# mgp25/OpenLTE

Measured on AMD Instinct MI355X. Metric: DL subframes/sec @20MHz 100RB 64QAM, full chain FFT->CE->demap->rate-unmatch->turbo(REF)->CRC (SURVEY 8d W4), higher is better.
Workload: dtype i8 IQ in, f32 FFT/CE/equaliser, i8 soft bits, i16 path metrics (differences exact modulo 2^16); 1 GPU; W4 full DL chain: 20 MHz/100 RB/64QAM, 9 allocations per subframe (8x12 PRB TBS 3240 + 1x4 PRB TBS 1064), 65536 subframes per GPU, int8 IQ in HBM; subframes_per_gpu=65536, N_ant=1, CFI=2, channel_estimate_form=compact, decoder=REF (reference-faithful, bit-exact), unique_subframes=96, streams_per_gpu=1

## Files before the change

### include/mi_lte.h

```cpp
#ifndef MI_LTE_H
#define MI_LTE_H

#include <stddef.h>
#include <stdint.h>

#ifdef __cplusplus
extern "C" {
#endif

#define MI_LTE_VERSION 100

typedef enum {
    MI_LTE_OK               = 0,
    MI_LTE_ERR_INVALID_ARG  = -1,
    MI_LTE_ERR_NO_DEVICE    = -2,
    MI_LTE_ERR_HIP          = -3,
    MI_LTE_ERR_UNSUPPORTED  = -4,
    MI_LTE_ERR_NOMEM        = -5
} mi_lte_status;

enum { MI_LTE_DECODE_SUCCESS = 0, MI_LTE_DECODE_INVALID_INPUTS = 1, MI_LTE_DECODE_FAIL = 2, MI_LTE_DECODE_INVALID_CRC = 3,
       MI_LTE_DECODE_INVALID_CONTENTS = 4 };

typedef struct mi_lte_ctx mi_lte_ctx;
// ... 53 lines not shown
    uint8_t  prb[2][112];
} mi_lte_pdsch_alloc;

typedef struct mi_lte_pdsch_plan mi_lte_pdsch_plan;
int      mi_lte_pdsch_plan_create(mi_lte_ctx *ctx, const mi_lte_dl_cfg *cfg, uint32_t N_pdcch_symbs,
                                  const mi_lte_pdsch_alloc *h_allocs, uint32_t n_alloc, mi_lte_pdsch_plan **out);
void     mi_lte_pdsch_plan_destroy(mi_lte_ctx *ctx, mi_lte_pdsch_plan *plan);
int      mi_lte_pdsch_plan_create_dynamic(mi_lte_ctx *ctx, const mi_lte_dl_cfg *cfg, uint32_t max_alloc, size_t max_soft_bytes,
                                          mi_lte_pdsch_plan **out);
int      mi_lte_pdsch_plan_assign(mi_lte_ctx *ctx, mi_lte_pdsch_plan *plan, uint32_t N_pdcch_symbs, const mi_lte_pdsch_alloc *h_allocs,
                                  uint32_t n_alloc);
uint32_t mi_lte_pdsch_plan_n_alloc(const mi_lte_pdsch_plan *plan);
int      mi_lte_pdsch_alloc_decodable(const mi_lte_dl_cfg *cfg, const mi_lte_pdsch_alloc *alloc, uint32_t N_pdcch_symbs);
int      mi_lte_pdsch_plan_set_decoder(mi_lte_pdsch_plan *plan, uint32_t mode , uint32_t n_iter, int qpp_spec);
int      mi_lte_pdsch_plan_set_output(mi_lte_pdsch_plan *plan, uint32_t packed);
uint32_t mi_lte_pdsch_plan_out_stride(const mi_lte_pdsch_plan *plan);
int      mi_lte_pdsch_decode_run(mi_lte_ctx *ctx, mi_lte_pdsch_plan *plan, const float *d_subframes,
                                 const uint32_t *d_subfr_num, const uint32_t *d_n_id_cell, uint8_t *d_out_bits,
                                 int32_t *d_status);
int      mi_lte_pdsch_plan_soft_bits(const mi_lte_pdsch_plan *plan, uint32_t alloc, const int8_t **d_e,
                                     const uint32_t **d_len);

typedef struct {
    uint32_t N_soft;
    uint32_t M_dl_harq;
} mi_lte_dlsch_cfg;

#define MI_LTE_DLSCH_MAX_CB 13
typedef struct {
    uint32_t C, K;
    uint32_t B;
    uint32_t N_cb, k0;
    uint32_t E[MI_LTE_DLSCH_MAX_CB];
    uint32_t off[MI_LTE_DLSCH_MAX_CB];
} mi_lte_dlsch_layout_t;

int mi_lte_dlsch_layout(uint32_t tbs, uint32_t G, uint32_t Q_m, uint32_t tx_mode, uint32_t rv, const mi_lte_dlsch_cfg *dlsch,
                        mi_lte_dlsch_layout_t *out);
int mi_lte_pdsch_plan_create_3gpp(mi_lte_ctx *ctx, const mi_lte_dl_cfg *cfg, uint32_t N_pdcch_symbs, const mi_lte_dlsch_cfg *dlsch,
                                  const mi_lte_pdsch_alloc *h_allocs, uint32_t n_alloc, mi_lte_pdsch_plan **out);
int mi_lte_pdsch_alloc_decodable_3gpp(const mi_lte_dl_cfg *cfg, const mi_lte_dlsch_cfg *dlsch, const mi_lte_pdsch_alloc *alloc,
                                      uint32_t N_pdcch_symbs);
int mi_lte_pdsch_plan_cb_soft(const mi_lte_pdsch_plan *plan, uint32_t alloc, const int8_t **d_blocks, uint32_t *C, uint32_t *K);
int mi_lte_pdsch_plan_cb_ok(const mi_lte_pdsch_plan *plan, const uint32_t **d_mask);

#define MI_LTE_DEMAP_REF    0u
#define MI_LTE_DEMAP_MAXLOG 1u
#define MI_LTE_DEMAP_AUTO_T 16
int mi_lte_pdsch_plan_set_demapper(mi_lte_pdsch_plan *plan, uint32_t mode, float gain);
int mi_lte_pdsch_plan_llr_gain(const mi_lte_pdsch_plan *plan, const float **d_gain);

typedef struct mi_lte_harq_pool mi_lte_harq_pool;
#define MI_LTE_HARQ_NONE     0xFFFFFFFFu
#define MI_LTE_HARQ_NEW_DATA 1u
typedef struct {
    uint32_t buf;
    uint32_t flags;
} mi_lte_harq_bind;
typedef struct {
    uint32_t tbs, C, K, N_cb;
    uint32_t n_tx;
    int32_t  status;
} mi_lte_harq_state;
size_t mi_lte_harq_buffer_bytes(uint32_t max_tbs);
int  mi_lte_harq_pool_create(mi_lte_ctx *ctx, uint32_t n_buf, uint32_t max_tbs, mi_lte_harq_pool **out);
void mi_lte_harq_pool_destroy(mi_lte_ctx *ctx, mi_lte_harq_pool *pool);
int  mi_lte_harq_pool_reset(mi_lte_ctx *ctx, mi_lte_harq_pool *pool, uint32_t buf);
int  mi_lte_pdsch_decode_run_harq(mi_lte_ctx *ctx, mi_lte_pdsch_plan *plan, mi_lte_harq_pool *pool, const mi_lte_harq_bind *h_bind,
                                  const float *d_subframes, const uint32_t *d_subfr_num, const uint32_t *d_n_id_cell, uint8_t *d_out_bits,
                                  int32_t *d_status);
int  mi_lte_harq_pool_soft(const mi_lte_harq_pool *pool, uint32_t buf, const int16_t **d_soft, const mi_lte_harq_state **d_state);

typedef enum { MI_LTE_TURBO_REF = 0, MI_LTE_TURBO_BCJR = 1, MI_LTE_TURBO_BCJR_BLOCK = 2, MI_LTE_TURBO_BCJR_EARLY = 3 } mi_lte_turbo_mode;
typedef enum { MI_LTE_SOFT_F32 = 0, MI_LTE_SOFT_I8 = 1, MI_LTE_SOFT_I16 = 2 } mi_lte_soft_type;

int mi_lte_turbo_decode_batch(mi_lte_ctx *ctx, const void *d_soft, mi_lte_soft_type soft_type, uint32_t K,
                              uint32_t n_cb, mi_lte_turbo_mode mode, uint32_t n_iter, int qpp_spec,
                              uint8_t *d_c_bits);

int mi_lte_turbo_early_exit_iterations(mi_lte_ctx *ctx, uint32_t *h_pair_iters, uint32_t max_pairs, uint32_t *n_pairs, uint32_t *n_iter);

int mi_lte_set_turbo_small_batch(mi_lte_ctx *ctx, uint32_t n_cb_max);
int mi_lte_set_turbo_merged(mi_lte_ctx *ctx, uint32_t on);

int mi_lte_rate_unmatch_turbo_batch(mi_lte_ctx *ctx, const float *d_e_bits, uint32_t N_e_bits, uint32_t D,
                                    uint32_t N_codeblocks, uint32_t tx_mode, uint32_t N_soft, uint32_t M_dl_harq,
                                    uint32_t chan_type, uint32_t rv_idx, uint32_t n_cb, float *d_d_bits);

size_t mi_lte_turbo_scratch_bytes(uint32_t K, uint32_t n_cb);
size_t mi_lte_turbo_bcjr_scratch_bytes(uint32_t K, uint32_t n_cb);

const char *mi_lte_last_kernels(const mi_lte_ctx *ctx);

size_t mi_lte_ul_subframe_floats(void);
int    mi_lte_ul_frontend_batch(mi_lte_ctx *ctx, const mi_lte_dl_cfg *cfg ,
                                const void *d_samples_a, const void *d_samples_b, const uint64_t *d_unit_start,
                                uint32_t n_units, float *d_subframes);

typedef struct {
    uint32_t group_assignment_pusch;
    uint32_t group_hopping_enabled;
    uint32_t sequence_hopping_enabled;
    uint32_t cyclic_shift;
    uint32_t cyclic_shift_dci;
} mi_lte_ul_cfg;

int mi_lte_ul_dmrs_pusch(const mi_lte_ul_cfg *ul, uint32_t N_id_cell, uint32_t N_subfr, uint32_t N_prb, float *h_dmrs_0_re,
                         float *h_dmrs_0_im, float *h_dmrs_1_re, float *h_dmrs_1_im);

typedef struct mi_lte_pusch_plan mi_lte_pusch_plan;
int      mi_lte_pusch_plan_create(mi_lte_ctx *ctx, const mi_lte_dl_cfg *cfg, const mi_lte_ul_cfg *ul,
                                  const uint32_t *h_unit_subfr_num, const uint32_t *h_unit_n_id_cell, uint32_t n_units,
                                  const mi_lte_pdsch_alloc *h_allocs, uint32_t n_alloc, mi_lte_pusch_plan **out);
void     mi_lte_pusch_plan_destroy(mi_lte_ctx *ctx, mi_lte_pusch_plan *plan);
uint32_t mi_lte_pusch_plan_out_stride(const mi_lte_pusch_plan *plan);
int      mi_lte_pusch_decode_run(mi_lte_ctx *ctx, mi_lte_pusch_plan *plan, const float *d_subframes, uint8_t *d_out_bits,
                                 int32_t *d_status);
int      mi_lte_pusch_plan_soft_bits(const mi_lte_pusch_plan *plan, uint32_t alloc, const int8_t **d_e, uint32_t *n_bits);

#define MI_LTE_ULSCH_N_SOFT 0xFFFFFFFFu
#define MI_LTE_ULSCH_M_HARQ 1u
int mi_lte_ulsch_layout(uint32_t tbs, uint32_t G, uint32_t Q_m, uint32_t rv, mi_lte_dlsch_layout_t *out);
int mi_lte_pusch_plan_create_3gpp(mi_lte_ctx *ctx, const mi_lte_dl_cfg *cfg, const mi_lte_ul_cfg *ul, const uint32_t *h_unit_subfr_num,
                                  const uint32_t *h_unit_n_id_cell, uint32_t n_units, const mi_lte_pdsch_alloc *h_allocs, uint32_t n_alloc,
                                  mi_lte_pusch_plan **out);
int mi_lte_pusch_plan_set_decoder(mi_lte_pusch_plan *plan, uint32_t mode, uint32_t n_iter, int qpp_spec);
int mi_lte_pusch_plan_set_output(mi_lte_pusch_plan *plan, uint32_t packed);
int mi_lte_pusch_plan_cb_soft(const mi_lte_pusch_plan *plan, uint32_t alloc, const int8_t **d_blocks, uint32_t *C, uint32_t *K);
int mi_lte_pusch_plan_cb_ok(const mi_lte_pusch_plan *plan, const uint32_t **d_mask);

typedef struct {
    uint8_t  O_ack, O_ri;
    uint16_t Qp_ack, Qp_ri;
    uint32_t Q_cqi;
} mi_lte_ulsch_uci;
enum { MI_LTE_UCI_ACK = 0, MI_LTE_UCI_RI = 1, MI_LTE_UCI_CQI = 2 };
int mi_lte_ulsch_uci_qprime(uint32_t kind, uint32_t O, uint32_t beta_x8, uint32_t M_sc_initial, uint32_t N_symb_initial, uint32_t sum_K_r,
                            uint32_t N_prb, uint32_t Qp_ri, uint32_t *Qp);
int mi_lte_ulsch_uci_G(uint32_t N_prb, uint32_t Q_m, const mi_lte_ulsch_uci *uci, uint32_t *G);
enum { MI_LTE_UCI_CELL_DATA = 0, MI_LTE_UCI_CELL_CQI = 1, MI_LTE_UCI_CELL_RI = 2, MI_LTE_UCI_CELL_ACK_DATA = 3, MI_LTE_UCI_CELL_ACK_CQI = 4 };
int mi_lte_ulsch_uci_map(uint32_t N_prb, uint32_t Q_m, const mi_lte_ulsch_uci *uci, uint8_t *kind , uint32_t *index );
typedef struct {
    uint8_t ack[2], ri[2];
    int32_t S_ack[3], S_ri[3];
} mi_lte_ulsch_uci_result;
int mi_lte_pusch_plan_create_3gpp_uci(mi_lte_ctx *ctx, const mi_lte_dl_cfg *cfg, const mi_lte_ul_cfg *ul, const uint32_t *h_unit_subfr_num,
                                      const uint32_t *h_unit_n_id_cell, uint32_t n_units, const mi_lte_pdsch_alloc *h_allocs, uint32_t n_alloc,
                                      const mi_lte_ulsch_uci *h_uci , mi_lte_pusch_plan **out);
int mi_lte_pusch_plan_uci_results(const mi_lte_pusch_plan *plan, const mi_lte_ulsch_uci_result **d_records);
int mi_lte_pusch_plan_cqi_soft(const mi_lte_pusch_plan *plan, uint32_t alloc, const int8_t **d_cqi, uint32_t *Q_cqi);
int mi_lte_pusch_plan_data_soft(const mi_lte_pusch_plan *plan, uint32_t alloc, const int8_t **d_data, uint32_t *G);

#define MI_LTE_CQI_MAX_BITS 128
enum { MI_LTE_CQI_NONE = 0, MI_LTE_CQI_NO_CRC = 1 , MI_LTE_CQI_CRC_OK = 2, MI_LTE_CQI_CRC_FAIL = 3 };
typedef struct {
    uint32_t O;
    uint32_t crc;
    int32_t  metric;
    int32_t  energy;
    uint32_t bits[4];
} mi_lte_cqi_result;
typedef struct { uint32_t off , Q_cqi, O, pad; } mi_lte_cqi_desc;
int mi_lte_cqi_encode(uint32_t O, const uint8_t *o_bits, uint32_t Q_cqi, uint8_t *q_bits );
int mi_lte_cqi_decode_batch(mi_lte_ctx *ctx, const int8_t *d_soft, const mi_lte_cqi_desc *d_desc, uint32_t n, mi_lte_cqi_result *d_out);
int mi_lte_pusch_plan_set_cqi_decode(mi_lte_pusch_plan *plan, const uint32_t *h_O_cqi );
int mi_lte_pusch_plan_cqi_results(const mi_lte_pusch_plan *plan, const mi_lte_cqi_result **d_records);
// ... 367 lines not shown
```

### openlte_amd/csrc/chain.hip

```cpp
#include <algorithm>
#include <cstring>
#include <type_traits>

#include "plan_core.hpp"
#include "phy_dev.hpp"
#include "demap_llr.h"

namespace {

constexpr int N_SC_MAX = 1200;

struct DemodGeom { uint32_t N_rb_dl, N_ant, cfi, sf_stride; };
__device__ __forceinline__ void sync_window(uint32_t N_rb_dl, uint32_t &first_sc, uint32_t &last_sc)
{
    switch (N_rb_dl) {
    case 6:  first_sc = 0;           last_sc = 71;          break;
    case 15: first_sc = 4 * 12 + 6;  last_sc = 11 * 12 - 7; break;
    case 25: first_sc = 9 * 12 + 6;  last_sc = 16 * 12 - 7; break;
    case 50: first_sc = 22 * 12;     last_sc = 28 * 12 - 1; break;
    case 75: first_sc = 34 * 12 + 6; last_sc = 41 * 12 - 7; break;
    default: first_sc = 47 * 12;     last_sc = 53 * 12 - 1; break;
    }
}
__device__ __forceinline__ uint32_t pdsch_mask(uint32_t N_ant, uint32_t cell, uint32_t sf, uint32_t L, uint32_t prb,
                                               uint32_t first_sc, uint32_t last_sc)
{
    const uint32_t l7 = L >= 7 ? L - 7 : L, c6 = cell % 6, c3 = cell % 3;
    uint32_t skip = 0;
    if (N_ant == 1) {
        if (l7 == 0) skip = 0x041u << c6;
        else if (l7 == 4) skip = 0x041u << ((c6 + 3) % 6);
    } else if (l7 == 0 || l7 == 4 || (N_ant == 4 && l7 == 1))
        skip = (0x249u << c3) & 0xFFFu;
    const bool win = (sf == 0 && L >= 7 && L <= 10) || ((sf == 0 || sf == 5) && (L == 5 || L == 6));
    const uint32_t s0 = prb * 12;
    if (win && last_sc >= s0 && first_sc <= s0 + 11) {
        const uint32_t lo = first_sc > s0 ? first_sc - s0 : 0u, hi = last_sc - s0 < 11u ? last_sc - s0 : 11u;
        skip |= ((2u << hi) - 1u) & ~((1u << lo) - 1u);
    }
    return ~skip & 0xFFFu;
}

__device__ __forceinline__ void pair_table_scan(uint2 *tab, const mi_lte_pdsch_alloc &al, uint32_t N_ant, uint32_t cell, uint32_t sf, uint32_t cfi,
                                                uint32_t n_pairs, uint32_t first_sc, uint32_t last_sc)
{
    const uint32_t N_prb = al.N_prb;
    const uint32_t ln = threadIdx.x, per = (n_pairs + 63) / 64, q0 = ln * per, q1 = min(q0 + per, n_pairs);
    const float r_prb = __builtin_amdgcn_rcpf((float)N_prb) * (1.0f + 0x1.8p-22f);
    uint32_t local = 0;
    for (uint32_t q = q0; q < q1; q++) {
        const uint32_t L = (uint32_t)((float)q * r_prb), prb = al.prb[L >= 7 ? 1 : 0][q - __umul24(L, N_prb)];
        const uint32_t m = L < cfi ? 0u : pdsch_mask(N_ant, cell, sf, L, prb, first_sc, last_sc);
        tab[q].y = m | ((L * N_SC_MAX + prb * 12) << 12);
        local += __popc(m);
    }
    uint32_t incl = local;
    for (int o = 1; o < 64; o <<= 1) {
        const uint32_t n = __shfl_up(incl, o);
        if ((int)ln >= o) incl += n;
    }
    uint32_t run = incl - local;
    for (uint32_t q = q0; q < q1; q++) {
        tab[q].x = run;
        run += __popc(tab[q].y & 0xFFFu);
    }
    if (ln == 63) tab[n_pairs] = make_uint2(incl, 0u);
}

template <bool ONE_PORT, bool COMPACT = false>
#ifndef DEMOD_WPE
#define DEMOD_WPE 8
#endif
#ifndef DEMOD_WPE_C
#define DEMOD_WPE_C 8
#endif
__global__ __launch_bounds__(256) __attribute__((amdgpu_waves_per_eu(COMPACT ? DEMOD_WPE_C : DEMOD_WPE, 8))) void k_pdsch_demod(const float *__restrict__ subframes, DemodGeom g,
                                                     const mi_lte_pdsch_alloc *__restrict__ allocs,
                                                     const uint32_t *__restrict__ subfr_num, const uint32_t *__restrict__ n_id_cell,
                                                     GoldTables gt, int8_t *__restrict__ e_base, const uint32_t *__restrict__ e_off,
                                                     uint32_t *__restrict__ e_len, uint32_t max_pairs, uint32_t max_words,
                                                     uint32_t e_lds_cap)
{
    extern __shared__ __attribute__((aligned(16))) uint32_t smu[];
    __shared__ uint2 qam_lut[64];
    const uint32_t a_idx = blockIdx.x;
    const mi_lte_pdsch_alloc &al = allocs[a_idx];
    const uint32_t unit = al.unit, sf = subfr_num[unit], cell = n_id_cell[unit], N_ant = ONE_PORT ? 1u : g.N_ant, N_prb = al.N_prb;
    const uint32_t Qm = al.mod_type == 3 ? 6 : al.mod_type == 2 ? 4 : al.mod_type == 1 ? 2 : 1;
    uint2    *tab = reinterpret_cast<uint2 *>(smu);
    uint32_t *cw  = smu + ((2 * (max_pairs + 1) + 3u) & ~3u);
    uint32_t first_sc, last_sc;
    sync_window(g.N_rb_dl, first_sc, last_sc);

    const uint32_t cfi = al.n_pdcch_symbs ? al.n_pdcch_symbs : g.cfi;
    const uint32_t n_pairs = 14 * N_prb, pair0 = cfi * N_prb;
    const uint32_t c_init = ((al.rnti << 14) | (0u << 13) | (sf << 9) | cell) & 0x7FFFFFFFu;
    if (threadIdx.x < 64) pair_table_scan(tab, al, N_ant, cell, sf, cfi, n_pairs, first_sc, last_sc);
    else {
        const uint32_t n_words_ub = ((n_pairs - pair0) * 12 * Qm + 31) / 32;
        if (threadIdx.x < 128) qam_lut[threadIdx.x - 64] = qam_lut_entry(threadIdx.x - 64);
        for (uint32_t w = threadIdx.x - 64; w <= n_words_ub; w += blockDim.x - 64) cw[w] = gold_word(gt, c_init, w);
    }
    __syncthreads();
    const uint32_t M_ap = tab[n_pairs].x;
    const uint32_t n_grp = M_ap >> (N_ant >> 1), M_symb = n_grp * N_ant, N_bits = M_symb * Qm;
    if (threadIdx.x == 0) e_len[a_idx] = N_bits;

    const float *base = subframes + (size_t)unit * g.sf_stride;
    const float *y_re_p = base, *y_im_p = base + 16 * N_SC_MAX;
    const float *h_re_p = base + 2 * 16 * N_SC_MAX, *h_im_p = h_re_p + (size_t)N_ant * 16 * N_SC_MAX;
    int8_t *e = e_base + (size_t)e_off[a_idx] * 64;
    auto locate = [&](uint32_t idx) -> uint32_t {
        uint32_t lo = pair0, hi = n_pairs;
        while (hi - lo > 1) {
            const uint32_t mid = (lo + hi) >> 1;
            if (tab[mid].x <= idx) lo = mid; else hi = mid;
        }
        const uint2 t = tab[lo];
        uint32_t r = idx - t.x, m = t.y & 0xFFFu;
        for (; r; r--) m &= m - 1;
        return (t.y >> 12) + (uint32_t)__builtin_ctz(m);
    };
    int8_t    *e_lds  = reinterpret_cast<int8_t *>(cw + max_words);
    const bool via_lds = N_bits <= e_lds_cap;
    auto run = [&](auto modc) {
    constexpr uint32_t MOD = decltype(modc)::value, QM = MOD == 3 ? 6 : MOD == 2 ? 4 : MOD == 1 ? 2 : 1;
    constexpr bool     QAM = MOD >= 2;
    auto put_bits = [&](auto *dst, uint32_t idx, const int8_t (&b)[6]) {
        const uint32_t n0 = idx * QM, w = n0 >> 5, sh = n0 & 31;
        const uint32_t c = __builtin_amdgcn_alignbit(cw[w + 1], cw[w], sh);
        if (QM == 1) dst[n0] = (c & 1u) ? (int8_t)-b[0] : b[0];
        else {
#pragma unroll
            for (uint32_t k = 0; k < 6; k += 2)
                if (k < QM) {
                    const int lo = ((c >> k) & 1u) ? -b[k] : b[k], hi = ((c >> (k + 1)) & 1u) ? -b[k + 1] : b[k + 1];
                    *reinterpret_cast<uint16_t *>(dst + n0 + k) = (uint16_t)((lo & 0xFF) | ((hi & 0xFF) << 8));
                }
        }
    };
    auto put_qam = [&](auto *dst, uint32_t idx, uint32_t neg) {
        const uint32_t n0 = QM == 4 ? idx << 2 : __umul24(idx, 6u), w = n0 >> 5, sh = n0 & 31;
        const uint32_t c  = __builtin_amdgcn_alignbit(cw[w + 1], cw[w], sh);
        const uint2    v  = qam_lut[(neg ^ c) & (QM == 4 ? 15u : 63u)];
        if (QM == 4) *reinterpret_cast<uint32_t *>(dst + n0) = v.x;
        else {
            *reinterpret_cast<uint16_t *>(dst + n0)     = (uint16_t)v.x;
            *reinterpret_cast<uint16_t *>(dst + n0 + 2) = (uint16_t)(v.x >> 16);
            *reinterpret_cast<uint16_t *>(dst + n0 + 4) = (uint16_t)v.y;
        }
    };
    auto put_symbol = [&](auto *dst, uint32_t idx, float nr, float ni, float den) {
        if constexpr (QAM) put_qam(dst, idx, qam_neg_bits_nodiv<MOD>(nr, ni, den));
        else {
            int8_t b[6] = {0, 0, 0, 0, 0, 0};
            demap_symbol<true>(nr / den, ni / den, MOD, b);
            put_bits(dst, idx, b);
        }
    };
    if (ONE_PORT && COMPACT) {
        constexpr uint32_t ROW = N_SC_MAX * 4, Y_IM = 16 * ROW, H_M = 32 * ROW, H_A = 48 * ROW;
        const uint32_t per_slot = N_prb * 12, n_items = 2 * per_slot;
        const auto rsrc = __builtin_amdgcn_make_buffer_rsrc(const_cast<float *>(base), 0, (int)(g.sf_stride * 4u), 0x00020000);
        auto ld = [&](uint32_t row, uint32_t off) { return __builtin_bit_cast(float, __builtin_amdgcn_raw_buffer_load_b32(rsrc, (int)off, (int)row, 0)); };
        auto body = [&](auto *dst) {
            for (uint32_t item = threadIdx.x; item < n_items; item += blockDim.x) {
                const uint32_t s = item >= per_slot ? 1u : 0u, r = item - s * per_slot, i = __umul24(r, 43691u) >> 19, j = r - ((i << 3) + (i << 2));
                const uint32_t bit = 1u << j, below = bit - 1u;
                const uint2   *tp = tab + (s ? 7 * N_prb : 0u) + i;
                const uint2    t0 = *tp;
                const uint32_t vy = ((t0.y >> 12) + j) << 2;
                const uint32_t vk = vy - s * (7 * ROW), vh = vk + s * (2 * ROW);
                const float M0 = ld(H_M, vh), M1 = ld(H_M + ROW, vh), M2 = ld(H_M + 2 * ROW, vh);
                const float P0 = ld(H_A, vh), P1 = ld(H_A + ROW, vh), P2 = ld(H_A + 2 * ROW, vh);
                const float Q0 = ld(H_A, vk), Q1 = ld(H_A + ROW, vk);
                float yr[7], yi[7];
#pragma unroll
                for (int t = 0; t < 7; t++) { yr[t] = ld(t * ROW, vy); yi[t] = ld(Y_IM + t * ROW, vy); }
                float m[7], a[7];
                m[0] = M0; a[0] = P0; m[4] = M1; a[4] = P1;
                float W0 = P0;
                if (s) W0 = wrap_phase_rare(P0, wrap_phase_rare(Q1, Q0));
                {
                    const float fm = (M1 - M0) / 4, W1 = wrap_phase_rare(P1, W0);
                    const float fa = wrap_phase_rare(W1 - W0, 0.0f) / 4;
                    float cm = M1, ca = W1;
#pragma unroll
                    for (int z = 3; z > 0; z--) { cm -= fm; ca -= fa; m[z] = cm; a[z] = ca; }
                    const float gm = div3(M2 - M1), W2 = wrap_phase_rare(P2, W1);
                    const float ga = div3(wrap_phase_rare(W2 - W1, 0.0f));
                    cm = M2; ca = W2;
#pragma unroll
                    for (int z = 6; z > 4; z--) { cm -= gm; ca -= ga; m[z] = cm; a[z] = ca; }
                }
#pragma unroll
                for (int t = 0; t < 7; t++) {
                    const uint2 pr = t ? tp[t * N_prb] : t0;
                    if (!(pr.y & bit)) continue;
                    const uint32_t idx = pr.x + __popc(pr.y & below);
                    float sn, cs;
                    ce_sincos(a[t], sn, cs);
                    const float mm = m[t], hr = mm * cs, hi = mm * sn;
                    const float hn = hr * hr + hi * hi;
                    put_symbol(dst, idx, yr[t] * hr + yi[t] * hi, yi[t] * hr - yr[t] * hi, hn);
                }
            }
        };
        if (via_lds) body(e_lds); else body(e);
    } else if (ONE_PORT) {
        constexpr int UNR = 4;
        const uint32_t q_thr = threadIdx.x / 12, j = threadIdx.x - 12 * q_thr, below = (1u << j) - 1u;
        const bool     lane_on = threadIdx.x < 252;
        auto body = [&](auto *dst) {
            for (uint32_t qb = pair0; qb < n_pairs; qb += 21 * UNR) {
                float    yr[UNR], yi[UNR], hr[UNR], hi[UNR];
                uint32_t idx[UNR];
                bool     on[UNR];
#pragma unroll
                for (int r = 0; r < UNR; r++) {
                    const uint32_t q = qb + 21 * r + q_thr;
                    const bool     in = lane_on && q < n_pairs;
                    const uint2    pr = tab[in ? q : 0u];
                    on[r]  = in && ((pr.y >> j) & 1u);
                    idx[r] = pr.x + __popc(pr.y & below);
                    const uint32_t ob = on[r] ? ((pr.y >> 12) + j) << 2 : 0u;
                    yr[r] = *reinterpret_cast<const float *>(reinterpret_cast<const char *>(y_re_p) + ob);
                    yi[r] = *reinterpret_cast<const float *>(reinterpret_cast<const char *>(y_im_p) + ob);
                    hr[r] = *reinterpret_cast<const float *>(reinterpret_cast<const char *>(h_re_p) + ob);
                    hi[r] = *reinterpret_cast<const float *>(reinterpret_cast<const char *>(h_im_p) + ob);
                }
#pragma unroll
                for (int r = 0; r < UNR; r++) {
                    if (!on[r]) continue;
                    const float hn = hr[r] * hr[r] + hi[r] * hi[r];
                    put_symbol(dst, idx[r], yr[r] * hr[r] + yi[r] * hi[r], yi[r] * hr[r] - yr[r] * hi[r], hn);
                }
            }
        };
        if (via_lds) body(e_lds); else body(e);
    } else
    for (uint32_t i = threadIdx.x; i < n_grp; i += blockDim.x) {
        float n_re[4], n_im[4], den[4];
        if (N_ant == 2) {
            const uint32_t p0 = locate(2 * i), p1 = locate(2 * i + 1);
            const float y0r = y_re_p[p0], y0i = y_im_p[p0], y1r = y_re_p[p1], y1i = y_im_p[p1];
            const float h0r = h_re_p[p0], h0i = h_im_p[p0], h1r = h_re_p[16 * N_SC_MAX + p0], h1i = h_im_p[16 * N_SC_MAX + p0];
            const float a0 = h0r * h0r + h0i * h0i, a1 = h1r * h1r + h1i * h1i;
            const float hn = sqrtf(a0 * a0 + a1 * a1);
            den[0] = den[1] = hn;
            n_re[0] = h0r * y0r + h0i * y0i + h1r * y1r + h1i * y1i;
            n_im[0] = h0r * y0i - h0i * y0r - h1r * y1i + h1i * y1r;
            n_re[1] = -h1r * y0r - h1i * y0i + h0r * y1r + h0i * y1i;
            n_im[1] = h1r * y0i - h1i * y0r + h0r * y1i - h0i * y1r;
        } else {
            const uint32_t p0 = locate(4 * i), p1 = locate(4 * i + 1), p2 = locate(4 * i + 2), p3 = locate(4 * i + 3);
            const size_t   ps = 16 * N_SC_MAX;
            const float y0r = y_re_p[p0], y0i = y_im_p[p0], y1r = y_re_p[p1], y1i = y_im_p[p1];
            const float y2r = y_re_p[p2], y2i = y_im_p[p2], y3r = y_re_p[p3], y3i = y_im_p[p3];
            const float h0r = h_re_p[p0], h0i = h_im_p[p0], h2r = h_re_p[2 * ps + p0], h2i = h_im_p[2 * ps + p0];
            const float h1r = h_re_p[ps + p2], h1i = h_im_p[ps + p2], h3r = h_re_p[3 * ps + p2], h3i = h_im_p[3 * ps + p2];
            const float a0 = h0r * h0r + h0i * h0i, a1 = h1r * h1r + h1i * h1i, a2 = h2r * h2r + h2i * h2i, a3 = h3r * h3r + h3i * h3i;
            const float n02 = sqrtf(a0 * a0 + a2 * a2), n13 = sqrtf(a1 * a1 + a3 * a3);
            den[0] = den[1] = n02; den[2] = den[3] = n13;
            n_re[0] = h0r * y0r + h0i * y0i + h2r * y1r + h2i * y1i;
            n_im[0] = h0r * y0i - h0i * y0r - h2r * y1i + h2i * y1r;
            n_re[1] = -h2r * y0r - h2i * y0i + h0r * y1r + h0i * y1i;
            n_im[1] = -(-h2r * y0i + h2i * y0r - h0r * y1i + h0i * y1r);
            n_re[2] = h1r * y2r + h1i * y2i + h3r * y3r + h3i * y3i;
            n_im[2] = h1r * y2i - h1i * y2r - h3r * y3i + h3i * y3r;
            n_re[3] = -h3r * y2r - h3i * y2i + h1r * y3r + h1i * y3i;
            n_im[3] = -(-h3r * y2i + h3i * y2r - h1r * y3i + h1i * y3r);
        }
        for (uint32_t p = 0; p < N_ant; p++) {
            if (via_lds) put_symbol(e_lds, i * N_ant + p, n_re[p], n_im[p], den[p]);
            else         put_symbol(e, i * N_ant + p, n_re[p], n_im[p], den[p]);
        }
    }
    };
    switch (al.mod_type) {
    case 0:  run(std::integral_constant<uint32_t, 0>{}); break;
    case 1:  run(std::integral_constant<uint32_t, 1>{}); break;
    case 2:  run(std::integral_constant<uint32_t, 2>{}); break;
    default: run(std::integral_constant<uint32_t, 3>{}); break;
    }
    if (via_lds) {
        __syncthreads();
        const uint32_t nq = (N_bits + 15) >> 4;
        for (uint32_t w = threadIdx.x; w < nq; w += blockDim.x) reinterpret_cast<uint4 *>(e)[w] = reinterpret_cast<const uint4 *>(e_lds)[w];
    }
}


__global__ __launch_bounds__(256) void k_pdsch_demod_llr(const float *__restrict__ subframes, DemodGeom g, const mi_lte_pdsch_alloc *__restrict__ allocs,
                                                         const uint32_t *__restrict__ subfr_num, const uint32_t *__restrict__ n_id_cell, GoldTables gt,
                                                         int8_t *__restrict__ e_base, const uint32_t *__restrict__ e_off, uint32_t *__restrict__ e_len,
                                                         uint32_t max_pairs, uint32_t max_words, uint32_t e_lds_cap, float gain, float auto_t,
                                                         float *__restrict__ llr_gain)
{
    extern __shared__ __attribute__((aligned(16))) uint32_t smu[];
    __shared__ double w_wave[4];
    const uint32_t a_idx = blockIdx.x;
    const mi_lte_pdsch_alloc &al = allocs[a_idx];
    const uint32_t unit = al.unit, sf = subfr_num[unit], cell = n_id_cell[unit], N_prb = al.N_prb;
    const uint32_t Qm = al.mod_type == 3 ? 6 : al.mod_type == 2 ? 4 : 2;
    uint2    *tab = reinterpret_cast<uint2 *>(smu);
    uint32_t *cw  = smu + ((2 * (max_pairs + 1) + 3u) & ~3u);
    uint32_t first_sc, last_sc;
    sync_window(g.N_rb_dl, first_sc, last_sc);
    const uint32_t cfi = al.n_pdcch_symbs ? al.n_pdcch_symbs : g.cfi;
    const uint32_t n_pairs = 14 * N_prb, pair0 = cfi * N_prb;
    const uint32_t c_init = ((al.rnti << 14) | (0u << 13) | (sf << 9) | cell) & 0x7FFFFFFFu;
    if (threadIdx.x < 64) pair_table_scan(tab, al, 1u, cell, sf, cfi, n_pairs, first_sc, last_sc);
    else {
        const uint32_t n_words_ub = ((n_pairs - pair0) * 12 * Qm + 31) / 32;
        for (uint32_t w = threadIdx.x - 64; w <= n_words_ub; w += blockDim.x - 64) cw[w] = gold_word(gt, c_init, w);
    }
    __syncthreads();
    const uint32_t M_symb = tab[n_pairs].x, N_bits = M_symb * Qm;
    if (threadIdx.x == 0) e_len[a_idx] = N_bits;

    const float *base = subframes + (size_t)unit * g.sf_stride;
    const char  *y_re_p = reinterpret_cast<const char *>(base), *y_im_p = y_re_p + 16 * N_SC_MAX * 4;
    const char  *h_re_p = y_im_p + 16 * N_SC_MAX * 4, *h_im_p = h_re_p + 16 * N_SC_MAX * 4;
    constexpr int  UNR = 4;
    const uint32_t q_thr = threadIdx.x / 12, j = threadIdx.x - 12 * q_thr, below = (1u << j) - 1u;
    const bool     lane_on = threadIdx.x < 252;
    auto element = [&](uint32_t q, uint32_t &ob, uint32_t &idx) __attribute__((always_inline)) -> bool {
        const bool  in = lane_on && q < n_pairs;
        const uint2 pr = tab[in ? q : 0u];
        const bool  on = in && ((pr.y >> j) & 1u);
        idx = pr.x + __popc(pr.y & below);
        ob  = on ? ((pr.y >> 12) + j) << 2 : 0u;
        return on;
    };
    double gd = (double)gain;
    if (gain == 0.0f) {
        double part = 0.0;
        for (uint32_t qb = pair0; qb < n_pairs; qb += 21 * UNR) {
            float hr[UNR], hi[UNR];
            bool  on[UNR];
#pragma unroll
            for (int r = 0; r < UNR; r++) {
                uint32_t ob, idx;
                on[r] = element(qb + 21 * r + q_thr, ob, idx);
                hr[r] = *reinterpret_cast<const float *>(h_re_p + ob);
                hi[r] = *reinterpret_cast<const float *>(h_im_p + ob);
            }
#pragma unroll
            for (int r = 0; r < UNR; r++)
                if (on[r]) part += (double)hr[r] * hr[r] + (double)hi[r] * hi[r];
        }
        for (int o = 32; o; o >>= 1) part += __shfl_xor(part, o);
        if ((threadIdx.x & 63u) == 0) w_wave[threadIdx.x >> 6] = part;
        __syncthreads();
        const double wbar = (((w_wave[0] + w_wave[1]) + w_wave[2]) + w_wave[3]) / (double)M_symb;
        const double a4 = al.mod_type == 3 ? 4.0 / 42 : al.mod_type == 2 ? 4.0 / 10 : 2.0;
        const float  gf = (float)((double)auto_t / (a4 * wbar));
        gd = (wbar > 0.0 && fabsf(gf) <= 3.4028234e38f) ? (double)gf : 0.0;
    }
    if (threadIdx.x == 0) llr_gain[a_idx] = (float)gd;

    int8_t    *e      = e_base + (size_t)e_off[a_idx] * 64;
    int8_t    *e_lds  = reinterpret_cast<int8_t *>(cw + max_words);
    const bool via_lds = N_bits <= e_lds_cap;
    auto run = [&](auto modc, auto *dst) __attribute__((always_inline)) {
        constexpr uint32_t MOD = decltype(modc)::value, QM = MOD == 3 ? 6 : MOD == 2 ? 4 : 2;
        for (uint32_t qb = pair0; qb < n_pairs; qb += 21 * UNR) {
            float    yr[UNR], yi[UNR], hr[UNR], hi[UNR];
            uint32_t idx[UNR];
            bool     on[UNR];
#pragma unroll
            for (int r = 0; r < UNR; r++) {
                uint32_t ob;
                on[r] = element(qb + 21 * r + q_thr, ob, idx[r]);
                yr[r] = *reinterpret_cast<const float *>(y_re_p + ob);
                yi[r] = *reinterpret_cast<const float *>(y_im_p + ob);
                hr[r] = *reinterpret_cast<const float *>(h_re_p + ob);
                hi[r] = *reinterpret_cast<const float *>(h_im_p + ob);
            }
#pragma unroll
            for (int r = 0; r < UNR; r++) {
                if (!on[r]) continue;
                const double Yr = yr[r], Yi = yi[r], Hr = hr[r], Hi = hi[r];
                const double w = Hr * Hr + Hi * Hi;
                double li[3], lq[3];
                llr_axis<MOD>(Yr * Hr + Yi * Hi, w, li);
                llr_axis<MOD>(Yi * Hr - Yr * Hi, w, lq);
                const uint32_t n0 = idx[r] * QM, c = __builtin_amdgcn_alignbit(cw[(n0 >> 5) + 1], cw[n0 >> 5], n0 & 31);
#pragma unroll
                for (uint32_t k = 0; k < QM; k += 2) {
                    const int vi = llr_byte(gd, li[k >> 1]), vq = llr_byte(gd, lq[k >> 1]);
                    const int lo = ((c >> k) & 1u) ? -vi : vi, hi8 = ((c >> (k + 1)) & 1u) ? -vq : vq;
                    *reinterpret_cast<uint16_t *>(dst + n0 + k) = (uint16_t)((lo & 0xFF) | ((hi8 & 0xFF) << 8));
                }
            }
        }
    };
    auto per_mod = [&](auto *dst) __attribute__((always_inline)) {
        switch (al.mod_type) {
        case 1:  run(std::integral_constant<uint32_t, 1>{}, dst); break;
        case 2:  run(std::integral_constant<uint32_t, 2>{}, dst); break;
        default: run(std::integral_constant<uint32_t, 3>{}, dst); break;
        }
    };
    if (via_lds) {
        per_mod(e_lds);
        __syncthreads();
        const uint32_t nq = (N_bits + 15) >> 4;
        for (uint32_t w = threadIdx.x; w < nq; w += blockDim.x) reinterpret_cast<uint4 *>(e)[w] = reinterpret_cast<const uint4 *>(e_lds)[w];
    } else
        per_mod(e);
}

}


struct mi_lte_pdsch_plan {
    mi_lte_dl_cfg cfg;
    MiPlanCore    core;
    uint32_t      decoder = MI_LTE_TURBO_REF, n_iter = 8;
    int           qpp_spec = 0;
    int8_t       *d_bcjr_soft = nullptr;
    uint8_t      *d_bcjr_bits = nullptr;
    size_t        bcjr_soft_cap = 0, bcjr_bits_cap = 0;
    uint32_t      cfi = 0, max_pairs = 0, max_words = 0, max_tbs = 0;
    bool          dynamic = false, wide = false;
    bool          mapped = false;
    void       *h_stage = nullptr;
    hipEvent_t  staged = nullptr;
    std::vector<uint8_t>  h_row;
    std::vector<uint32_t> h_e_bits;
    MiDlsch3   *g3 = nullptr;
    uint32_t    demap = MI_LTE_DEMAP_REF;
    float       demap_gain = 0.0f, *d_llr_gain = nullptr;
};

static void plan_set_stride(mi_lte_pdsch_plan *pl)
{
    pl->core.out_stride = mi_out_stride((pl->dynamic || pl->wide) ? 6120u : pl->max_tbs, pl->core.packed != 0);
}

static int plan_layout(mi_lte_ctx *ctx, mi_lte_pdsch_plan *pl, uint32_t N_pdcch_symbs, const mi_lte_pdsch_alloc *h_allocs, uint32_t n_alloc,
                       std::vector<uint32_t> *cb_alloc, bool prbs_checked = false)
{
    std::vector<uint8_t>  &row    = pl->h_row;
    std::vector<uint32_t> &e_bits = pl->h_e_bits;
    row.resize(n_alloc);
    e_bits.resize(n_alloc);
    const mi_lte_dl_cfg *cfg = &pl->cfg;
    pl->cfi          = N_pdcch_symbs;
    pl->core.n_alloc = n_alloc;
    pl->max_pairs = pl->max_words = pl->max_tbs = 0;
    pl->core.groups.clear();
    for (uint32_t a = 0; a < n_alloc; a++) {
        const mi_lte_pdsch_alloc &al = h_allocs[a];
        const int      r   = cb_alloc ? mi_qpp_row_at_least(al.tbs + 24) : 0;
        const uint32_t cfi = al.n_pdcch_symbs ? al.n_pdcch_symbs : N_pdcch_symbs;
        if (r < 0 || al.N_prb == 0 || al.N_prb > cfg->N_rb_dl || al.mod_type > 3 || cfi < 1 || cfi > 4) {
            ctx->err = "allocation outside the single-code-block envelope (tbs + 24 > 6144) or malformed";
            return MI_LTE_ERR_UNSUPPORTED;
        }
        for (uint32_t s = 0; s < 2 && !prbs_checked; s++)
            for (uint32_t i = 0; i < al.N_prb; i++)
                if (al.prb[s][i] >= cfg->N_rb_dl) {
                    ctx->err = "allocation names a resource block outside the carrier";
                    return MI_LTE_ERR_INVALID_ARG;
                }
        row[a]      = (uint8_t)r;
        pl->max_tbs = std::max(pl->max_tbs, al.tbs);
        const uint32_t Qm = al.mod_type == 3 ? 6 : al.mod_type == 2 ? 4 : al.mod_type == 1 ? 2 : 1;
        const uint32_t pairs = (14 - cfi) * al.N_prb, e_max = pairs * 12 * Qm;
        pl->max_pairs = std::max(pl->max_pairs, 14 * al.N_prb);
        pl->max_words = std::max(pl->max_words, (e_max + 31) / 32);
        e_bits[a]     = e_max;
    }
    if (pl->max_words > 4095) {
        ctx->err = "allocation larger than the scrambling table";
        return MI_LTE_ERR_UNSUPPORTED;
    }
    pl->core.e_bytes = mi_plan_soft_layout(e_bits.data(), n_alloc, pl->core.h_e_off);
    plan_set_stride(pl);
    if (cb_alloc) mi_plan_group(row.data(), nullptr, e_bits.data(), n_alloc, pl->core.groups, *cb_alloc);
    return MI_LTE_OK;
}

extern "C" {

void mi_lte_pdsch_plan_destroy(mi_lte_ctx *ctx, mi_lte_pdsch_plan *pl);

int mi_lte_pdsch_plan_create(mi_lte_ctx *ctx, const mi_lte_dl_cfg *cfg, uint32_t N_pdcch_symbs,
                             const mi_lte_pdsch_alloc *h_allocs, uint32_t n_alloc, mi_lte_pdsch_plan **out)
{
    if (!ctx || !cfg || !h_allocs || !out || n_alloc == 0 || N_pdcch_symbs < 1 || N_pdcch_symbs > 4) return MI_LTE_ERR_INVALID_ARG;
    if (!(cfg->N_ant == 1 || cfg->N_ant == 2 || cfg->N_ant == 4)) return MI_LTE_ERR_INVALID_ARG;
    if ((cfg->sample_format & MI_LTE_CE_COMPACT) && cfg->N_ant != 1) { ctx->err = "MI_LTE_CE_COMPACT: single-port cells only"; return MI_LTE_ERR_UNSUPPORTED; }
    MI_HIP_CHECK(ctx, hipSetDevice(ctx->device));
    auto *pl      = new mi_lte_pdsch_plan();
    auto  guard   = on_fail([&] { (void)hipStreamSynchronize(ctx->stream); mi_lte_pdsch_plan_destroy(nullptr, pl); });
    pl->cfg       = *cfg;
    std::vector<uint32_t> cb_alloc;
    int rc = plan_layout(ctx, pl, N_pdcch_symbs, h_allocs, n_alloc, &cb_alloc);
    if (rc != MI_LTE_OK) return rc;
    MI_HIP_CHECK(ctx, pl->core.allocate(n_alloc, pl->core.e_bytes));
    MI_H2D(ctx, pl->core.d_allocs, h_allocs, sizeof(mi_lte_pdsch_alloc) * n_alloc);
    MI_H2D(ctx, pl->core.d_e_off, pl->core.h_e_off.data(), sizeof(uint32_t) * n_alloc);
    MI_H2D(ctx, pl->core.d_cb_alloc, cb_alloc.data(), sizeof(uint32_t) * n_alloc);
    MI_HIP_CHECK(ctx, mi_stream_wait_polling(ctx));
    guard.armed = false;
    *out = pl;
    return MI_LTE_OK;
}

int mi_lte_pdsch_plan_create_dynamic(mi_lte_ctx *ctx, const mi_lte_dl_cfg *cfg, uint32_t max_alloc, size_t max_soft_bytes, mi_lte_pdsch_plan **out)
{
    if (!ctx || !cfg || !out || max_alloc == 0) return MI_LTE_ERR_INVALID_ARG;
    if (!(cfg->N_ant == 1 || cfg->N_ant == 2 || cfg->N_ant == 4)) return MI_LTE_ERR_INVALID_ARG;
    if ((cfg->sample_format & MI_LTE_CE_COMPACT) && cfg->N_ant != 1) { ctx->err = "MI_LTE_CE_COMPACT: single-port cells only"; return MI_LTE_ERR_UNSUPPORTED; }
    MI_HIP_CHECK(ctx, hipSetDevice(ctx->device));
    auto *pl    = new mi_lte_pdsch_plan();
    auto  guard = on_fail([&] { mi_lte_pdsch_plan_destroy(nullptr, pl); });
    pl->cfg     = *cfg;
    pl->dynamic = true;
    max_alloc = (max_alloc + 3u) & ~3u;
    MI_HIP_CHECK(ctx, pl->core.allocate(max_alloc, (max_soft_bytes + 63) & ~(size_t)63));
    MI_HIP_CHECK(ctx, hipHostMalloc(&pl->h_stage, (sizeof(mi_lte_pdsch_alloc) + 2 * sizeof(uint32_t)) * (size_t)max_alloc, hipHostMallocDefault));
    MI_HIP_CHECK(ctx, hipEventCreateWithFlags(&pl->staged, hipEventDisableTiming));
    guard.armed = false;
    *out = pl;
    return MI_LTE_OK;
}
}

int mi_pdsch_plan_create_mapped(mi_lte_ctx *ctx, const mi_lte_dl_cfg *cfg, uint32_t max_alloc, size_t max_soft_bytes, mi_lte_pdsch_plan **out)
{
    if (!ctx || !cfg || !out || max_alloc == 0 || max_alloc > 64) return MI_LTE_ERR_INVALID_ARG;
    if (!(cfg->N_ant == 1 || cfg->N_ant == 2 || cfg->N_ant == 4) || (cfg->sample_format & MI_LTE_CE_COMPACT)) return MI_LTE_ERR_INVALID_ARG;
    MI_HIP_CHECK(ctx, hipSetDevice(ctx->device));
    auto *pl    = new mi_lte_pdsch_plan();
    auto  guard = on_fail([&] { mi_lte_pdsch_plan_destroy(nullptr, pl); });
    pl->cfg     = *cfg;
    pl->dynamic = pl->mapped = true;
    MI_HIP_CHECK(ctx, hipHostMalloc(&pl->h_stage, (sizeof(mi_lte_pdsch_alloc) + 2 * sizeof(uint32_t)) * (size_t)max_alloc, hipHostMallocMapped | hipHostMallocCoherent));
    void *d_stage = nullptr;
    MI_HIP_CHECK(ctx, hipHostGetDevicePointer(&d_stage, pl->h_stage, 0));
    MI_HIP_CHECK(ctx, pl->core.allocate(max_alloc, (max_soft_bytes + 63) & ~(size_t)63, d_stage));
    guard.armed = false;
    *out = pl;
    return MI_LTE_OK;
}

static bool alloc_geometry_ok(const mi_lte_dl_cfg *cfg, const mi_lte_pdsch_alloc *al, uint32_t N_pdcch_symbs)
{
    const uint32_t cfi = al->n_pdcch_symbs ? al->n_pdcch_symbs : N_pdcch_symbs;
    if (al->N_prb == 0 || al->N_prb > cfg->N_rb_dl || al->N_prb > 110 || al->mod_type > 3 || cfi < 1 || cfi > 4) return false;
    if ((14 - cfi) * al->N_prb * 12 * (al->mod_type == 3 ? 6u : al->mod_type == 2 ? 4u : al->mod_type == 1 ? 2u : 1u) > 4095u * 32u) return false;
    for (uint32_t s = 0; s < 2; s++)
// ... 76 lines not shown
    memcpy(so, pl->core.h_e_off.data(), sizeof(uint32_t) * n_alloc);
    memcpy(sc, cb_alloc.data(), sizeof(uint32_t) * n_alloc);
    if (pl->mapped) return MI_LTE_OK;
    MI_HIP_CHECK(ctx, hipMemcpyAsync(pl->core.d_allocs, sa, sizeof(mi_lte_pdsch_alloc) * n_alloc, hipMemcpyHostToDevice, ctx->stream));
    MI_HIP_CHECK(ctx, hipMemcpyAsync(pl->core.d_e_off, so, sizeof(uint32_t) * n_alloc, hipMemcpyHostToDevice, ctx->stream));
    MI_HIP_CHECK(ctx, hipMemcpyAsync(pl->core.d_cb_alloc, sc, sizeof(uint32_t) * n_alloc, hipMemcpyHostToDevice, ctx->stream));
    MI_HIP_CHECK(ctx, hipEventRecord(pl->staged, ctx->stream));
    return MI_LTE_OK;
}

uint32_t mi_lte_pdsch_plan_n_alloc(const mi_lte_pdsch_plan *pl) { return pl ? pl->core.n_alloc : 0; }
}

int mi_pdsch_plan_assign_slice(mi_lte_ctx *ctx, mi_lte_pdsch_plan *pl, uint32_t N_pdcch_symbs, const mi_lte_pdsch_alloc *h_src, uint32_t n_alloc, uint32_t unit0,
                               std::vector<uint32_t> *refused, hipStream_t copy_stream)
{
    if (!ctx || !pl || !pl->dynamic || pl->mapped || !h_src || n_alloc == 0 || N_pdcch_symbs < 1 || N_pdcch_symbs > 4) return MI_LTE_ERR_INVALID_ARG;
    const hipStream_t cs = copy_stream ? copy_stream : ctx->stream;
    if (n_alloc > pl->core.cap_alloc) { ctx->err = "more allocations than the dynamic plan was created for"; return MI_LTE_ERR_INVALID_ARG; }
    MI_HIP_CHECK(ctx, hipSetDevice(ctx->device));
    MI_HIP_CHECK(ctx, hipEventSynchronize(pl->staged));
    auto *sa = (mi_lte_pdsch_alloc *)pl->h_stage;
    auto *so = (uint32_t *)(sa + pl->core.cap_alloc), *sc = so + pl->core.cap_alloc;
    for (uint32_t i = 0; i < n_alloc; i++) {
        mi_lte_pdsch_alloc &a = sa[i];
        a = h_src[i];
        a.unit -= unit0;
        if (!mi_lte_pdsch_alloc_decodable(&pl->cfg, &a, N_pdcch_symbs)) {
            a.N_prb = 1; a.prb[0][0] = a.prb[1][0] = 0; a.mod_type = 1; a.tbs = 16; a.rv_idx = 0; a.tx_mode = pl->cfg.N_ant == 1 ? 1 : 2;
            if (a.n_pdcch_symbs > 4) a.n_pdcch_symbs = 0;
            if (refused) refused->push_back(i);
        }
    }
    std::vector<uint32_t> cb_alloc;
    int rc = plan_layout(ctx, pl, N_pdcch_symbs, sa, n_alloc, &cb_alloc, true);
    if (rc != MI_LTE_OK) { pl->core.n_alloc = 0; return rc; }
    if (pl->core.e_bytes > pl->core.cap_e_bytes) { pl->core.n_alloc = 0; ctx->err = "more soft bits than the dynamic plan was created for"; return MI_LTE_ERR_INVALID_ARG; }
    memcpy(so, pl->core.h_e_off.data(), sizeof(uint32_t) * n_alloc);
    memcpy(sc, cb_alloc.data(), sizeof(uint32_t) * n_alloc);
    static const bool slice_by_engine = getenv("MI_LTE_SLICE_COPY_COMMANDS") != nullptr;
    if (slice_by_engine) {
        MI_HIP_CHECK(ctx, hipMemcpyAsync(pl->core.d_allocs, sa, sizeof(mi_lte_pdsch_alloc) * n_alloc, hipMemcpyHostToDevice, cs));
        MI_HIP_CHECK(ctx, hipMemcpyAsync(pl->core.d_e_off, so, sizeof(uint32_t) * n_alloc, hipMemcpyHostToDevice, cs));
        MI_HIP_CHECK(ctx, hipMemcpyAsync(pl->core.d_cb_alloc, sc, sizeof(uint32_t) * n_alloc, hipMemcpyHostToDevice, cs));
    } else {
        const MiCopySeg segs[3] = {{pl->core.d_allocs, sa, sizeof(mi_lte_pdsch_alloc) * n_alloc}, {pl->core.d_e_off, so, sizeof(uint32_t) * n_alloc}, {pl->core.d_cb_alloc, sc, sizeof(uint32_t) * n_alloc}};
        MI_HIP_CHECK(ctx, mi_pinned_segments_to_device(ctx, segs, 3, cs));
    }
    MI_HIP_CHECK(ctx, hipEventRecord(pl->staged, cs));
    return MI_LTE_OK;
}
void mi_pdsch_plan_wide_stride(mi_lte_pdsch_plan *pl) { pl->wide = true; plan_set_stride(pl); }
extern "C" {

void mi_lte_pdsch_plan_destroy(mi_lte_ctx *ctx, mi_lte_pdsch_plan *pl)
{
    if (!pl) return;
    if (ctx) {
        (void)hipSetDevice(ctx->device);
        (void)hipStreamSynchronize(ctx->stream);
    }
    pl->core.release();
    if (pl->d_bcjr_soft) (void)hipFree(pl->d_bcjr_soft);
    if (pl->d_bcjr_bits) (void)hipFree(pl->d_bcjr_bits);
    if (pl->d_llr_gain) (void)hipFree(pl->d_llr_gain);
    if (pl->h_stage) (void)hipHostFree(pl->h_stage);
    if (pl->staged) (void)hipEventDestroy(pl->staged);
    mi_dlsch3_free(pl->g3);
    delete pl;
}

uint32_t mi_lte_pdsch_plan_out_stride(const mi_lte_pdsch_plan *pl) { return pl ? pl->core.out_stride : 0; }

int mi_lte_model_atan2f(const float *h_y, const float *h_x, float *h_out, size_t n)
{
    if (!h_y || !h_x || !h_out) return MI_LTE_ERR_INVALID_ARG;
    for (size_t i = 0; i < n; i++) h_out[i] = ref_atan2f(h_y[i], h_x[i]);
    return MI_LTE_OK;
}

int mi_lte_pdsch_plan_soft_bits(const mi_lte_pdsch_plan *pl, uint32_t alloc, const int8_t **d_e, const uint32_t **d_len)
{
    if (!pl || alloc >= pl->core.n_alloc || !d_e || !d_len) return MI_LTE_ERR_INVALID_ARG;
    *d_e   = pl->core.d_e + (size_t)pl->core.h_e_off[alloc] * 64;
    *d_len = pl->core.d_e_len + alloc;
    return MI_LTE_OK;
}

int mi_lte_pdsch_plan_set_decoder(mi_lte_pdsch_plan *pl, uint32_t mode, uint32_t n_iter, int qpp_spec)
{
    const bool bcjr = mi_is_bcjr(mode);
    if (!pl || !(mode == MI_LTE_TURBO_REF || bcjr) || (bcjr && (n_iter == 0 || n_iter > 64))) return MI_LTE_ERR_INVALID_ARG;
    if (pl->g3 && mode == MI_LTE_TURBO_REF) return MI_LTE_ERR_UNSUPPORTED;
    if (pl->g3 && !qpp_spec) return MI_LTE_ERR_INVALID_ARG;
    pl->decoder = mode; pl->n_iter = n_iter; pl->qpp_spec = qpp_spec;
    return MI_LTE_OK;
}

int mi_lte_pdsch_plan_set_demapper(mi_lte_pdsch_plan *pl, uint32_t mode, float gain)
{
    if (!pl || mode > MI_LTE_DEMAP_MAXLOG) return MI_LTE_ERR_INVALID_ARG;
    if (mode == MI_LTE_DEMAP_REF) { pl->demap = MI_LTE_DEMAP_REF; return MI_LTE_OK; }
    if (!(gain >= 0.0f) || gain > 3.4028234e38f) return MI_LTE_ERR_INVALID_ARG;
    if (!pl->g3 || (pl->cfg.sample_format & MI_LTE_CE_COMPACT)) return MI_LTE_ERR_UNSUPPORTED;
    pl->demap = mode; pl->demap_gain = gain;
    return MI_LTE_OK;
}

int mi_lte_pdsch_plan_llr_gain(const mi_lte_pdsch_plan *pl, const float **d_gain)
{
    if (!pl || !d_gain || !pl->d_llr_gain) return MI_LTE_ERR_INVALID_ARG;
    *d_gain = pl->d_llr_gain;
    return MI_LTE_OK;
}

int mi_lte_pdsch_plan_set_output(mi_lte_pdsch_plan *pl, uint32_t packed)
{
    if (!pl) return MI_LTE_ERR_INVALID_ARG;
    pl->core.packed = packed ? 1u : 0u;
    plan_set_stride(pl);
    return MI_LTE_OK;
}

}

static int pdsch_demod(mi_lte_ctx *ctx, mi_lte_pdsch_plan *pl, const float *d_subframes, const uint32_t *d_subfr_num, const uint32_t *d_n_id_cell)
{
    MI_HIP_CHECK(ctx, hipSetDevice(ctx->device));
    int rc = mi_ctx_gold_tables(ctx);
    if (rc != MI_LTE_OK) return rc;
    DemodGeom  g{pl->cfg.N_rb_dl, pl->cfg.N_ant, pl->cfi, (uint32_t)mi_lte_subframe_floats(pl->cfg.N_ant)};
    GoldTables gt{ctx->d_gold_x1, ctx->d_gold_x2b, ctx->gold_words};
    const uint32_t words_al = (pl->max_words + 1u + 3u) & ~3u, e_bytes = (pl->max_words * 32 + 63u) & ~63u;
    const uint32_t e_cap = (e_bytes <= 32 * 1024) ? e_bytes : 0;
    const uint32_t pairs_al = ((2 * (pl->max_pairs + 1) + 3u) & ~3u);
    const size_t lds = sizeof(uint32_t) * ((size_t)pairs_al + words_al) + e_cap;
    uint32_t threads = 256;
    if (const char *ev = getenv("MI_LTE_PDSCH_THREADS")) {
        const int t = atoi(ev);
        if (t >= 64 && t <= 256 && t % 64 == 0) threads = (uint32_t)t;
    }
    auto launch = [&](auto kernel) {
        MI_LAUNCH(ctx, "k_pdsch_demod", kernel, dim3(pl->core.n_alloc), dim3(threads), lds, d_subframes, g, pl->core.d_allocs, d_subfr_num, d_n_id_cell, gt,
                  pl->core.d_e, pl->core.d_e_off, pl->core.d_e_len, pl->max_pairs, words_al, e_cap);
    };
    if (pl->demap == MI_LTE_DEMAP_MAXLOG) {
        float auto_t = (float)MI_LTE_DEMAP_AUTO_T;
        if (const char *ev = getenv("MI_LTE_DEMAP_AUTO_T")) {
            const float t = (float)atof(ev);
            if (t >= 1.0f && t <= 127.0f) auto_t = t;
        }
        MI_LAUNCH(ctx, "k_pdsch_demod_llr", k_pdsch_demod_llr, dim3(pl->core.n_alloc), dim3(256), lds, d_subframes, g, pl->core.d_allocs, d_subfr_num,
                  d_n_id_cell, gt, pl->core.d_e, pl->core.d_e_off, pl->core.d_e_len, pl->max_pairs, words_al, e_cap, pl->demap_gain, auto_t, pl->d_llr_gain);
    } else if (g.N_ant == 1 && (pl->cfg.sample_format & MI_LTE_CE_COMPACT)) launch(k_pdsch_demod<true, true>);
    else if (g.N_ant == 1) launch(k_pdsch_demod<true>);
    else launch(k_pdsch_demod<false>);
    MI_HIP_CHECK(ctx, hipGetLastError());
    return MI_LTE_OK;
}

static int pdsch_run(mi_lte_ctx *ctx, mi_lte_pdsch_plan *pl, mi_lte_harq_pool *pool, const mi_lte_harq_bind *h_bind, const float *d_subframes,
                     const uint32_t *d_subfr_num, const uint32_t *d_n_id_cell, uint8_t *d_out_bits, int32_t *d_status)
{
    if (!ctx || !pl || !d_subframes || !d_subfr_num || !d_n_id_cell || !d_out_bits || !d_status) return MI_LTE_ERR_INVALID_ARG;
    int rc;
    if (pool) {
        if (!pl->g3) { ctx->err = "HARQ soft combining needs a plan in the 3GPP transport-block mode"; return MI_LTE_ERR_UNSUPPORTED; }
        if ((rc = mi_dlsch3_harq_check(ctx, pl->g3, pool, h_bind)) != MI_LTE_OK) return rc;
    }
    if (pl->core.n_alloc == 0) { ctx->err = "the dynamic plan holds no allocations (mi_lte_pdsch_plan_assign)"; return MI_LTE_ERR_INVALID_ARG; }
    if ((rc = pdsch_demod(ctx, pl, d_subframes, d_subfr_num, d_n_id_cell)) != MI_LTE_OK) return rc;
    const MiDecodeIO io = pl->core.io(d_out_bits, d_status, false);
    if (pl->g3) {
        rc = mi_dlsch3_run(ctx, pl->g3, pool, h_bind, io, pl->decoder, pl->n_iter);
        if (rc == MI_LTE_OK && pl->demap == MI_LTE_DEMAP_MAXLOG) ctx->last_kernels.replace(0, strlen("k_pdsch_demod"), "k_pdsch_demod_llr");
        return rc;
    }
    if (!mi_is_bcjr(pl->decoder)) {
        rc = mi_turbo_ref_dispatch(ctx, pl->core.groups.data(), (uint32_t)pl->core.groups.size(), io, &pl->core.multi);
        if (rc != MI_LTE_OK) return rc;
        ctx->last_kernels.insert(0, "k_pdsch_demod:1,");
        return MI_LTE_OK;
    }
    size_t soft = 0, bits = 0;
    for (auto &gr : pl->core.groups) { soft = std::max(soft, (size_t)gr.n_cb * 3 * (gr.K + 4)); bits = std::max(bits, (size_t)gr.n_cb * gr.K); }
    if (soft > pl->bcjr_soft_cap || bits > pl->bcjr_bits_cap) {
        MI_HIP_CHECK(ctx, hipStreamSynchronize(ctx->stream));
        if (pl->d_bcjr_soft) (void)hipFree(pl->d_bcjr_soft);
        if (pl->d_bcjr_bits) (void)hipFree(pl->d_bcjr_bits);
        pl->d_bcjr_soft = nullptr; pl->d_bcjr_bits = nullptr;
        MI_HIP_CHECK(ctx, hipMalloc((void **)&pl->d_bcjr_soft, soft));
        MI_HIP_CHECK(ctx, hipMalloc((void **)&pl->d_bcjr_bits, bits));
        pl->bcjr_soft_cap = soft; pl->bcjr_bits_cap = bits;
    }
    for (auto &gr : pl->core.groups) {
        rc = mi_turbo_bcjr_group(ctx, gr, io, pl->d_bcjr_soft, pl->d_bcjr_bits, pl->decoder, pl->n_iter, pl->qpp_spec);
        if (rc != MI_LTE_OK) return rc;
    }
    ctx->last_kernels = pl->decoder == MI_LTE_TURBO_BCJR_BLOCK ? "k_pdsch_demod:1,k_rm_to_i8,k_bcjr_block,k_crc_finish per block size"
                                                               : "k_pdsch_demod:1,k_cb_desc,k_rm_bcjr_prep,k_bcjr_half,k_bcjr_final,k_crc_finish per block size";
    return MI_LTE_OK;
}

extern "C" {

int mi_lte_pdsch_decode_run(mi_lte_ctx *ctx, mi_lte_pdsch_plan *pl, const float *d_subframes, const uint32_t *d_subfr_num,
                            const uint32_t *d_n_id_cell, uint8_t *d_out_bits, int32_t *d_status)
{
    return pdsch_run(ctx, pl, nullptr, nullptr, d_subframes, d_subfr_num, d_n_id_cell, d_out_bits, d_status);
}

int mi_lte_pdsch_decode_run_harq(mi_lte_ctx *ctx, mi_lte_pdsch_plan *pl, mi_lte_harq_pool *pool, const mi_lte_harq_bind *h_bind, const float *d_subframes,
                                 const uint32_t *d_subfr_num, const uint32_t *d_n_id_cell, uint8_t *d_out_bits, int32_t *d_status)
{
    if (!pool || !h_bind) return MI_LTE_ERR_INVALID_ARG;
    return pdsch_run(ctx, pl, pool, h_bind, d_subframes, d_subfr_num, d_n_id_cell, d_out_bits, d_status);
}

}
```

### openlte_amd/csrc/ctx.cc

```cpp
#include <cmath>

#include <chrono>
#include <cstdlib>

#include <algorithm>

#include "ctx.hpp"
#include "build_id.h"

#include <cstring>

#include "lte_tables.h"

extern "C" {

int mi_lte_version(void) { return MI_LTE_VERSION; }
const char *mi_lte_build_id(void) { return MI_LTE_BUILD_ID; }

int mi_lte_device_count(void)
{
    int n = 0;
    if (hipGetDeviceCount(&n) != hipSuccess) return 0;
    return n;
}

int mi_lte_ctx_create(int device, mi_lte_ctx **out)
{
    if (!out) return MI_LTE_ERR_INVALID_ARG;
    *out  = nullptr;
    int n = mi_lte_device_count();
    if (n <= 0 || device < 0 || device >= n) {
        fprintf(stderr, "mi_lte: no usable HIP device %d (found %d); this library has no CPU fallback\n", device, n);
        return MI_LTE_ERR_NO_DEVICE;
    }
    mi_lte_ctx *ctx = new mi_lte_ctx();
    ctx->device     = device;
    if (const char *e = getenv("MI_LTE_NO_MERGED_DECODE")) ctx->merged_decode = atoi(e) == 0;
    hipDeviceProp_t prop;
    if (hipSetDevice(device) != hipSuccess || hipGetDeviceProperties(&prop, device) != hipSuccess) {
        delete ctx;
        return MI_LTE_ERR_HIP;
    }
    ctx->dev_name = std::string(prop.name) + " (" + prop.gcnArchName + ")";
    if (std::strncmp(prop.gcnArchName, "gfx950", 6) != 0) {
        fprintf(stderr, "mi_lte: device %d is %s, but the kernels are built for gfx950 only\n", device, prop.gcnArchName);
        delete ctx;
        return MI_LTE_ERR_NO_DEVICE;
    }
    if (hipStreamCreateWithFlags(&ctx->stream, hipStreamNonBlocking) != hipSuccess || hipEventCreate(&ctx->ev0) != hipSuccess ||
        hipEventCreate(&ctx->ev1) != hipSuccess) {
        delete ctx;
        return MI_LTE_ERR_HIP;
    }
    *out = ctx;
    return MI_LTE_OK;
}

void mi_lte_ctx_destroy(mi_lte_ctx *ctx)
{
    if (!ctx) return;
    (void)hipSetDevice(ctx->device);
    (void)hipStreamSynchronize(ctx->stream);
    if (ctx->host_cache_free) ctx->host_cache_free(ctx);
    for (void *p : ctx->owned) (void)hipFree(p);
    for (hipEvent_t e : ctx->prof_pool) (void)hipEventDestroy(e);
    if (ctx->scratch) (void)hipFree(ctx->scratch);
    if (ctx->h_small) (void)hipHostFree(ctx->h_small);
    if (ctx->h_bounce) (void)hipHostFree(ctx->h_bounce);
    for (int k = 0; k < 2; k++)
        if (ctx->ev_bounce[k]) (void)hipEventDestroy(ctx->ev_bounce[k]);
    if (ctx->h_flag) (void)hipHostFree(ctx->h_flag);
    if (ctx->ev0) (void)hipEventDestroy(ctx->ev0);
    if (ctx->ev1) (void)hipEventDestroy(ctx->ev1);
    if (ctx->stream) (void)hipStreamDestroy(ctx->stream);
    delete ctx;
}

int mi_lte_set_turbo_small_batch(mi_lte_ctx *ctx, uint32_t n_cb_max)
{
    if (!ctx) return MI_LTE_ERR_INVALID_ARG;
    ctx->siso_small_max = n_cb_max;
    return MI_LTE_OK;
}

int mi_lte_set_turbo_merged(mi_lte_ctx *ctx, uint32_t on)
{
    if (!ctx) return MI_LTE_ERR_INVALID_ARG;
    ctx->merged_decode = on != 0;
    return MI_LTE_OK;
}

const char *mi_lte_last_error(const mi_lte_ctx *ctx) { return ctx ? ctx->err.c_str() : "null context"; }
const char *mi_lte_device_name(const mi_lte_ctx *ctx) { return ctx ? ctx->dev_name.c_str() : ""; }
void       *mi_lte_stream(const mi_lte_ctx *ctx) { return ctx ? (void *)ctx->stream : nullptr; }
const char *mi_lte_last_kernels(const mi_lte_ctx *ctx) { return ctx ? ctx->last_kernels.c_str() : ""; }

int mi_lte_malloc(mi_lte_ctx *ctx, size_t bytes, void **d_ptr)
{
    if (!ctx || !d_ptr) return MI_LTE_ERR_INVALID_ARG;
    MI_HIP_CHECK(ctx, hipSetDevice(ctx->device));
    MI_HIP_CHECK(ctx, hipMalloc(d_ptr, bytes ? bytes : 1));
    return MI_LTE_OK;
}
int mi_lte_free(mi_lte_ctx *ctx, void *d_ptr)
{
    if (!ctx) return MI_LTE_ERR_INVALID_ARG;
    MI_HIP_CHECK(ctx, hipSetDevice(ctx->device));
    MI_HIP_CHECK(ctx, hipStreamSynchronize(ctx->stream));
    MI_HIP_CHECK(ctx, hipFree(d_ptr));
    return MI_LTE_OK;
}
int mi_lte_memset(mi_lte_ctx *ctx, void *d_ptr, int value, size_t bytes)
{
    if (!ctx) return MI_LTE_ERR_INVALID_ARG;
    MI_HIP_CHECK(ctx, hipMemsetAsync(d_ptr, value, bytes, ctx->stream));
    return MI_LTE_OK;
}
}
namespace {
typedef uint32_t mi_u32x4 __attribute__((ext_vector_type(4)));
template <bool NT> __global__ void k_copy16(const mi_u32x4 *__restrict__ src, mi_u32x4 *__restrict__ dst, size_t n)
{
    const size_t i = (size_t)blockIdx.x * blockDim.x + threadIdx.x;
    if (i >= n) return;
    if (NT) __builtin_nontemporal_store(__builtin_nontemporal_load(src + i), dst + i);
    else dst[i] = src[i];
}
__global__ void k_copy16_loop(const mi_u32x4 *__restrict__ src, mi_u32x4 *__restrict__ dst, size_t n)
{
    for (size_t i = (size_t)blockIdx.x * blockDim.x + threadIdx.x; i < n; i += (size_t)gridDim.x * blockDim.x) dst[i] = src[i];
}
}
extern "C" {
int mi_lte_device_copy_rate(mi_lte_ctx *ctx, size_t bytes, uint32_t reps, double *gb_per_s)
{
    if (!ctx || !gb_per_s || bytes < 16 || (bytes & 15) || reps == 0) return MI_LTE_ERR_INVALID_ARG;
    MI_HIP_CHECK(ctx, hipSetDevice(ctx->device));
    mi_u32x4 *a = nullptr, *b = nullptr;
    auto      guard = on_fail([&] { (void)hipStreamSynchronize(ctx->stream); (void)hipFree(a); (void)hipFree(b); });
    MI_HIP_CHECK(ctx, hipMalloc((void **)&a, bytes));
    MI_HIP_CHECK(ctx, hipMalloc((void **)&b, bytes));
    MI_HIP_CHECK(ctx, hipMemsetAsync(a, 0x5A, bytes, ctx->stream));
    const size_t n = bytes / 16;
    if ((n + 255) / 256 > 0x7FFFFFFFull) return MI_LTE_ERR_INVALID_ARG;
    const dim3 block(256), grid_all((unsigned)((n + 255) / 256)), grid_loop((unsigned)std::min<size_t>((n + 255) / 256, 256 * 32));
    double     best = 0.0;
    for (int shape = 0; shape < 3; shape++) {
        auto launch = [&](const mi_u32x4 *s, mi_u32x4 *d) {
            if (shape == 0) hipLaunchKernelGGL(k_copy16<false>, grid_all, block, 0, ctx->stream, s, d, n);
            else if (shape == 1) hipLaunchKernelGGL(k_copy16<true>, grid_all, block, 0, ctx->stream, s, d, n);
            else hipLaunchKernelGGL(k_copy16_loop, grid_loop, block, 0, ctx->stream, s, d, n);
        };
        launch(a, b);
        MI_HIP_CHECK(ctx, hipEventRecord(ctx->ev0, ctx->stream));
        for (uint32_t r = 0; r < reps; r++) launch((r & 1) ? b : a, (r & 1) ? a : b);
        MI_HIP_CHECK(ctx, hipEventRecord(ctx->ev1, ctx->stream));
        MI_HIP_CHECK(ctx, hipEventSynchronize(ctx->ev1));
        MI_HIP_CHECK(ctx, hipGetLastError());
        float ms = 0.f;
        MI_HIP_CHECK(ctx, hipEventElapsedTime(&ms, ctx->ev0, ctx->ev1));
        const double r = 2.0 * (double)bytes * reps / ((double)ms * 1e-3) / 1e9;
        ctx->copy_rates[shape] = r;
        best = std::max(best, r);
    }
    *gb_per_s = best;
    guard.armed = false;
    (void)hipFree(a); (void)hipFree(b);
    return MI_LTE_OK;
}
int mi_lte_device_copy_rates(const mi_lte_ctx *ctx, double *out3)
{
// ... 417 lines not shown
```

### openlte_amd/csrc/ctx.hpp

```cpp
#pragma once

#include <hip/hip_runtime.h>

#include <cstdint>
#include <cstdio>
#include <map>
#include <string>
#include <vector>

#include "../../include/mi_lte.h"
#include "turbo_plan.hpp"

struct TurboTables {
    uint16_t *d_pi  = nullptr;
    uint16_t *d_inv = nullptr;
    uint16_t *d_inv2 = nullptr;
    uint32_t *d_pi_row = nullptr, *d_inv_row = nullptr;
};

struct RmTables {
    uint16_t *d_tabs = nullptr;
    uint32_t *d_nnn  = nullptr;
};

enum : uint32_t { MI_FFT_TWC_P2 = 0, MI_FFT_TWC_P3 = 32, MI_FFT_TWC_L2048 = 288, MI_FFT_TWC_L1024 = 1312, MI_FFT_TWC_L256 = 1824, MI_FFT_TWC_L128 = 1952,
                  MI_FFT_TWC_X2 = 2016, MI_FFT_TWC_X3 = 2048,
                  MI_FFT_TWC_TOTAL = 2560 };

constexpr uint32_t MI_CRC_TAB_BIAS = 8;

struct mi_lte_ctx {
    int                device = -1;
    hipStream_t        stream = nullptr;
    hipEvent_t         ev0 = nullptr, ev1 = nullptr;
    std::string        err;
    std::string        dev_name;
    std::string        last_kernels;
    double             copy_rates[3] = {0, 0, 0};
    void              *scratch       = nullptr;
    size_t             scratch_bytes = 0;
    uint32_t          *h_flag = nullptr, *d_flag = nullptr;
    uint32_t           flag_seq = 0;
    uint32_t *bcjr_early_buf = nullptr; size_t bcjr_early_cap = 0;
    struct { uint32_t *chg; uint32_t n_pairs, n_iter, n_cb; } bcjr_early = {nullptr, 0, 0, 0};
    bool               bcjr_block_lds_set = false;
    uint32_t           siso_small_max = 4096;
    bool               merged_decode = true;
    void              *h_small = nullptr, *d_small = nullptr;
    void              *h_bounce = nullptr, *d_bounce = nullptr;
    hipEvent_t         ev_bounce[2] = {nullptr, nullptr};
    bool               bounce_failed = false;
    std::map<uint64_t, TurboTables> turbo_tables;
    std::map<uint32_t, RmTables>    rm_tables;
    std::vector<void *> owned;

    uint32_t *d_gold_x1 = nullptr, *d_gold_x2b = nullptr;
    uint32_t  gold_words = 0;
    void     *d_pusch_shapes = nullptr;

    float2   *d_fft_tw  = nullptr;
    uint32_t *d_crc_tab = nullptr;
    float2   *d_prach_tab = nullptr;
    float2   *d_prach_tab4 = nullptr;

    bool                                   prof_on = false, prof_armed = false;
    std::vector<hipEvent_t>                prof_pool;
    size_t                                 prof_used = 0;
    std::vector<std::pair<const char *, size_t>> prof_recs;
    std::string                            prof_report;

    void *host_cache = nullptr;
    void (*host_cache_free)(mi_lte_ctx *) = nullptr;
};

void mi_prof_begin(mi_lte_ctx *ctx, const char *name);
void mi_prof_end(mi_lte_ctx *ctx);

#define MI_LAUNCH(ctx, name, kernel, grid, block, shmem, ...)                                         \
    do {                                                                                             \
        mi_prof_begin((ctx), (name));                                                                \
        hipLaunchKernelGGL(kernel, grid, block, shmem, (ctx)->stream, __VA_ARGS__);                  \
        mi_prof_end((ctx));                                                                          \
    } while (0)

#define MI_HIP_CHECK(ctx, call)                                                                      \
    do {                                                                                             \
        hipError_t e_ = (call);                                                                      \
        if (e_ != hipSuccess) {                                                                      \
            (ctx)->err = std::string(#call) + ": " + hipGetErrorString(e_);                          \
            return MI_LTE_ERR_HIP;                                                                   \
        }                                                                                            \
    } while (0)

#define MI_H2D(ctx, d, h, n) do { const int rc_ = mi_lte_memcpy_h2d((ctx), (d), (h), (n)); if (rc_ != MI_LTE_OK) return rc_; } while (0)
#define MI_D2H(ctx, h, d, n) do { const int rc_ = mi_lte_memcpy_d2h((ctx), (h), (d), (n)); if (rc_ != MI_LTE_OK) return rc_; } while (0)

template <typename F> struct OnFail {
    F    f;
    bool armed = true;
    ~OnFail() { if (armed) f(); }
};
template <typename F> OnFail<F> on_fail(F f) { return OnFail<F>{f}; }

int   mi_ctx_reserve_scratch(mi_lte_ctx *ctx, size_t bytes);
hipError_t mi_pinned_to_device(mi_lte_ctx *ctx, void *d_dst, const void *h_pinned, size_t bytes, hipStream_t stream = nullptr);
hipError_t mi_device_to_pinned(mi_lte_ctx *ctx, void *h_pinned, const void *d_src, size_t bytes);
struct MiCopySeg { void *dst; const void *src; size_t bytes; };
hipError_t mi_pinned_segments_to_device(mi_lte_ctx *ctx, const MiCopySeg *segs, uint32_t n_seg, hipStream_t stream);
constexpr size_t MI_SMALL_BYTES = 64 * 1024;
int   mi_ctx_small_results(mi_lte_ctx *ctx, size_t bytes, void **h, void **d);
hipError_t mi_stream_wait(mi_lte_ctx *ctx, size_t n_units);
hipError_t mi_stream_wait_polling(mi_lte_ctx *ctx);
int   mi_ctx_gold_tables(mi_lte_ctx *ctx);
int   mi_ctx_crc_table(mi_lte_ctx *ctx);
int   mi_ctx_fft_twiddles(mi_lte_ctx *ctx);
struct MiMultiCache { void *d_tab = nullptr; size_t cap = 0; std::vector<MiKGroup> built_for; MiMultiGeom geom; };
void  mi_multi_cache_free(MiMultiCache *cache);
int   mi_ctx_turbo_tables(mi_lte_ctx *ctx, uint32_t K, int spec, TurboTables *out);
struct mi_lte_pdsch_plan;
int   mi_pdsch_plan_create_mapped(mi_lte_ctx *ctx, const mi_lte_dl_cfg *cfg, uint32_t max_alloc, size_t max_soft_bytes, mi_lte_pdsch_plan **out);
int   mi_pdsch_plan_assign_slice(mi_lte_ctx *ctx, mi_lte_pdsch_plan *pl, uint32_t N_pdcch_symbs, const mi_lte_pdsch_alloc *h_src, uint32_t n_alloc, uint32_t unit0,
                                 std::vector<uint32_t> *refused, hipStream_t copy_stream = nullptr);
void  mi_pdsch_plan_wide_stride(mi_lte_pdsch_plan *pl);
constexpr uint32_t MI_PUCCH_STAGED_MAX = 32;
struct MiPucchStaged { char *h_base = nullptr, *d_base = nullptr; size_t o_tab = 0, o_out = 0; uint32_t n_res = 0; };
int   mi_pucch_stage(mi_lte_ctx *ctx, uint32_t N_rb_ul, const mi_lte_pucch_res *h_res, const float *h_tables, uint32_t n_res, MiPucchStaged *st);
int   mi_pucch_launch(mi_lte_ctx *ctx, const MiPucchStaged *st, uint32_t N_rb_ul, const float *d_subframes);
void  mi_pucch_collect(const MiPucchStaged *st, uint8_t *h_bits, uint32_t *h_n_bits, uint32_t *h_rc);
struct mi_lte_pusch_plan;
int   mi_pusch_plan_create_impl(mi_lte_ctx *ctx, const mi_lte_dl_cfg *cfg, const mi_lte_ul_cfg *ul, const uint32_t *h_unit_subfr_num,
// ... 10 lines not shown
```

### openlte_amd/csrc/plan_core.hpp

```cpp
#pragma once

#include "ctx.hpp"

int mi_qpp_row_at_least(uint32_t B);

inline uint32_t mi_out_stride(uint32_t tbs, bool packed) { return packed ? (((tbs + 7) / 8 + 63) & ~63u) : ((tbs + 63) & ~63u); }
inline bool     mi_is_bcjr(uint32_t mode) { return mode == MI_LTE_TURBO_BCJR || mode == MI_LTE_TURBO_BCJR_BLOCK || mode == MI_LTE_TURBO_BCJR_EARLY; }

size_t mi_plan_soft_layout(const uint32_t *e_bits, uint32_t n_alloc, std::vector<uint32_t> &h_e_off);

void mi_plan_group(const uint8_t *row, const uint32_t *n_cb, const uint32_t *e_bits, uint32_t n_alloc, std::vector<MiKGroup> &groups, std::vector<uint32_t> &slot_alloc);

struct MiDecodeIO {
    const mi_lte_pdsch_alloc *d_allocs;
    const uint32_t *d_cb_alloc, *d_e_off, *d_e_len;
    const int8_t   *d_e;
    uint8_t        *d_out_bits;
    int32_t        *d_status;
    uint32_t        out_stride;
    bool            ul, packed;
};

struct MiPlanCore {
    uint32_t n_alloc = 0, out_stride = 0, packed = 0;
    size_t   e_bytes = 0;
    uint32_t cap_alloc = 0;
    size_t   cap_e_bytes = 0;
    mi_lte_pdsch_alloc *d_allocs = nullptr;
    uint32_t *d_e_off = nullptr, *d_e_len = nullptr, *d_cb_alloc = nullptr;
    int8_t   *d_e = nullptr;
    bool      desc_views = false;
    std::vector<MiKGroup> groups;
    std::vector<uint32_t> h_e_off;
    MiMultiCache          multi;

    hipError_t allocate(uint32_t n_alloc_max, size_t e_bytes_max, void *d_desc_block = nullptr);
    void       release();
    MiDecodeIO io(uint8_t *d_out_bits, int32_t *d_status, bool ul) const { return {d_allocs, d_cb_alloc, d_e_off, d_e_len, d_e, d_out_bits, d_status, out_stride, ul, packed != 0}; }
};

int   mi_turbo_ref_dispatch(mi_lte_ctx *ctx, const MiKGroup *groups, uint32_t n_groups, const MiDecodeIO &io, MiMultiCache *cache);
int   mi_turbo_bcjr_group(mi_lte_ctx *ctx, const MiKGroup &gr, const MiDecodeIO &io, int8_t *d_soft, uint8_t *d_c_bits, uint32_t mode, uint32_t n_iter, int qpp_spec);

struct MiDlsch3;
int             mi_dlsch3_create(mi_lte_ctx *ctx, const mi_lte_dlsch_cfg *cfg, const mi_lte_pdsch_alloc *h_allocs, uint32_t n_alloc, MiDlsch3 **out);
void            mi_dlsch3_free(MiDlsch3 *g);
int             mi_dlsch3_run(mi_lte_ctx *ctx, MiDlsch3 *g, mi_lte_harq_pool *p, const mi_lte_harq_bind *h_bind, const MiDecodeIO &io, uint32_t decoder, uint32_t n_iter);
int             mi_dlsch3_cb_soft(const MiDlsch3 *g, uint32_t alloc, const int8_t **d_blocks, uint32_t *C, uint32_t *K);
const uint32_t *mi_dlsch3_cb_ok(const MiDlsch3 *g);
int             mi_dlsch3_harq_check(mi_lte_ctx *ctx, const MiDlsch3 *g, const mi_lte_harq_pool *p, const mi_lte_harq_bind *h_bind);
```

### openlte_amd/csrc/turbo.hip

```cpp
#include <algorithm>
#include <cstring>
#include <initializer_list>
#include <type_traits>
#include <vector>

#include "plan_core.hpp"
#include "turbo_swar.h"

using namespace turbo_geom;

namespace {

constexpr uint32_t RX_NULL_AS_INT = 10000;


__device__ __forceinline__ int sbyte(uint32_t w, int k) { return (int)__builtin_amdgcn_sbfe(w, 8 * k, 8); }

typedef __attribute__((address_space(3))) const uint8_t  lds_u8_t;
typedef __attribute__((address_space(3))) const int8_t   lds_i8_t;
typedef __attribute__((address_space(3))) const uint16_t lds_u16_t;
__device__ __forceinline__ uint32_t lds_u8(uint32_t addr) { return *(lds_u8_t *)(uintptr_t)addr; }
__device__ __forceinline__ int      lds_i8(uint32_t addr) { return *(lds_i8_t *)(uintptr_t)addr; }
__device__ __forceinline__ uint32_t lds_u16(uint32_t addr) { return *(lds_u16_t *)(uintptr_t)addr; }

typedef short v2s __attribute__((ext_vector_type(2)));
__device__ __forceinline__ v2s      as_v2s(uint32_t w) { return __builtin_bit_cast(v2s, w); }
__device__ __forceinline__ uint32_t as_u32(v2s v) { return __builtin_bit_cast(uint32_t, v); }
__device__ __forceinline__ uint32_t neg_mask(v2s d)
{
    uint32_t m;
    asm("v_pk_ashrrev_i16 %0, 15, %1 op_sel_hi:[0,1]" : "=v"(m) : "v"(as_u32(d)));
    return m;
}
__device__ __forceinline__ v2s bit_select(uint32_t m, v2s yes, v2s no) { return as_v2s((as_u32(yes) & m) | (as_u32(no) & ~m)); }
__device__ __forceinline__ int soft_xor(int a, int b)
{
    int mag = (abs(a) + abs(b)) >> 1;
    return ((a < 0) != (b < 0)) ? -mag : mag;
}


template <typename Op> __device__ __forceinline__ int wave_reduce_i(int v, Op op)
{
    v = op(v, __builtin_amdgcn_update_dpp(v, v, 0xB1, 0xF, 0xF, false));
    v = op(v, __builtin_amdgcn_update_dpp(v, v, 0x4E, 0xF, 0xF, false));
    v = op(v, __builtin_amdgcn_update_dpp(v, v, 0x141, 0xF, 0xF, false));
    v = op(v, __builtin_amdgcn_update_dpp(v, v, 0x140, 0xF, 0xF, false));
    return op(op(__builtin_amdgcn_readlane(v, 0), __builtin_amdgcn_readlane(v, 16)), op(__builtin_amdgcn_readlane(v, 32), __builtin_amdgcn_readlane(v, 48)));
}
__device__ __forceinline__ int      wave_max_i(int v) { return wave_reduce_i(v, [](int a, int b) { return max(a, b); }); }
__device__ __forceinline__ uint32_t wave_xor_u(uint32_t v) { return (uint32_t)wave_reduce_i((int)v, [](int a, int b) { return a ^ b; }); }
__device__ __forceinline__ float    wave_max_f(float v)
{
    return __int_as_float(wave_max_i(__float_as_int(v)));
}

__device__ __forceinline__ float block_max_abs_f(float v, float *red )
{
    v = wave_max_f(v);
    __syncthreads();
    if ((threadIdx.x & 63) == 0) red[threadIdx.x >> 6] = v;
    __syncthreads();
    float r = red[0];
    for (uint32_t w = 1; w < (blockDim.x >> 6); w++) r = fmaxf(r, red[w]);
    return r;
}
__device__ __forceinline__ int block_max_i(int v, int *red)
{
    v = wave_max_i(v);
    __syncthreads();
    if ((threadIdx.x & 63) == 0) red[threadIdx.x >> 6] = v;
    __syncthreads();
    int r = red[0];
    for (uint32_t w = 1; w < (blockDim.x >> 6); w++) r = max(r, red[w]);
    return r;
}

__device__ __forceinline__ void block_max_i2(int &a, int &b, int *red)
{
    a = wave_max_i(a); b = wave_max_i(b);
    __syncthreads();
    if ((threadIdx.x & 63) == 0) { red[threadIdx.x >> 6] = a; red[8 + (threadIdx.x >> 6)] = b; }
    __syncthreads();
    a = red[0]; b = red[8];
    for (uint32_t w = 1; w < (blockDim.x >> 6); w++) { a = max(a, red[w]); b = max(b, red[8 + w]); }
}

struct PrepOut { uint8_t *arr[6]; };

__device__ __forceinline__ uint4 pack16(const int (&q)[16])
// ... 64 lines not shown
#pragma unroll
                for (int k = 0; k < 4; k++) put(4 * w + k, (float)sbyte(x, k));
            }
        } else if (sizeof(T) == 2) {
            const uint4 *g = reinterpret_cast<const uint4 *>(p);
#pragma unroll
            for (int w = 0; w < 6; w++) {
                const uint4    x = (w < 3 || nvalid > 8) ? g[w] : make_uint4(0, 0, 0, 0);
                const uint32_t c[4] = {x.x, x.y, x.z, x.w};
#pragma unroll
                for (int k = 0; k < 8; k++) put(8 * w + k, (float)(int)__builtin_amdgcn_sbfe(c[k >> 1], 16 * (k & 1), 16));
            }
        } else {
            const float4 *g = reinterpret_cast<const float4 *>(p);
#pragma unroll
            for (int w = 0; w < 12; w++) {
                const float4 x = (w < 6 || nvalid > 8) ? g[w] : make_float4(0, 0, 0, 0);
                put(4 * w, x.x); put(4 * w + 1, x.y); put(4 * w + 2, x.z); put(4 * w + 3, x.w);
            }
        }
    }
};

struct RmGeom {
    uint32_t R, K_pi, N_d, N_cb, k0m, Nnn, cnt_k0, mask0, mask2;
    __device__ __forceinline__ static uint32_t lowmask(uint32_t n) { return n >= 32 ? 0xFFFFFFFFu : ((1u << n) - 1u); }
    __device__ __forceinline__ uint32_t nulls_below(uint32_t p) const
    {
        if (p <= K_pi) return __popc(mask0 & lowmask((p + R - 1) / R));
        const uint32_t q = p - K_pi, a = (q + 1) >> 1, b = q >> 1;
        return __popc(mask0) + __popc(mask0 & lowmask((a + R - 1) / R)) + __popc(mask2 & lowmask((b + R - 1) / R)) +
               ((b > K_pi - 1) ? 1u : 0u);
    }
    __device__ __forceinline__ uint32_t cnt(uint32_t p) const { return p - nulls_below(p); }
    __device__ __forceinline__ void init(uint32_t D, uint32_t tx_mode, uint32_t rv, uint32_t N_soft = 250368,
                                         uint32_t M_dl_harq = 8, uint32_t C = 1, bool limited = true)
    {
        R    = (D + 31) / 32;
        K_pi = 32 * R;
        N_d  = K_pi - D;
        const uint32_t K_w = 3 * K_pi, K_mimo = (tx_mode == 3 || tx_mode == 4 || tx_mode == 8 || tx_mode == 9) ? 2 : 1;
        const uint32_t N_ir = N_soft / (K_mimo * (M_dl_harq < 8 ? M_dl_harq : 8));
        N_cb = (limited && N_ir / C < K_w) ? N_ir / C : K_w;
        const uint32_t k0 = R * (2 * ((N_cb + 8 * R - 1) / (8 * R)) * rv + 2);
        k0m  = k0 % N_cb;
        mask0 = mask2 = 0;
        for (uint32_t c = 0; c < 32; c++) {
            const uint32_t P = __brev(c) >> 27;
            if (P < N_d) mask0 |= 1u << c;
            if (P + 1 < N_d) mask2 |= 1u << c;
        }
        Nnn    = cnt(N_cb);
        cnt_k0 = cnt(k0m);
    }
    __device__ __forceinline__ uint32_t pos(uint32_t i, int x) const
    {
        const uint32_t n = i + N_d;
        if (x == 2) {
            const uint32_t m = n - 1, ii = (__brev(m & 31) >> 27) * R + (m >> 5);
            return K_pi + 2 * ii + 1;
        }
        const uint32_t ii = (__brev(n & 31) >> 27) * R + (n >> 5);
        return x == 0 ? ii : K_pi + 2 * ii;
    }
    __device__ __forceinline__ void pos_cnt(uint32_t i, int x, uint32_t &p, uint32_t &cn) const
    {
        const uint32_t n = i + N_d - (x == 2 ? 1u : 0u), c = __brev(n & 31) >> 27, r = n >> 5, ii = c * R + r;
        const uint32_t cc = c + (r > 0 ? 1u : 0u);
        uint32_t nulls;
        if (x == 0) {
            p     = ii;
            nulls = __popc(mask0 & lowmask(cc));
        } else if (x == 1) {
            p     = K_pi + 2 * ii;
            nulls = __popc(mask0) + __popc(mask0 & lowmask(cc)) + __popc(mask2 & lowmask(cc));
        } else {
            p     = K_pi + 2 * ii + 1;
            nulls = __popc(mask0) + __popc(mask0 & lowmask(c + 1)) + __popc(mask2 & lowmask(cc));
        }
        cn = p - nulls;
    }
};

struct CbDesc { uint32_t alloc, e_off, E, combo, Nnn, hard, tbs, pad; };

struct GroupDesc {
    const mi_lte_pdsch_alloc *allocs;
    const uint32_t *cb_alloc;
    const int8_t   *e_base;
    const uint32_t *e_off;
    const uint32_t *e_len;
    uint8_t        *out_bits;
    uint32_t        out_stride;
    int32_t        *status;
    const uint32_t *crc_tab;
    uint32_t        ul;
    uint32_t        packed;
    const CbDesc   *desc;
};

typedef __attribute__((address_space(4))) const KSeg     const_seg_t;
typedef __attribute__((address_space(4))) const uint32_t const_map_t;
__device__ __forceinline__ const_seg_t &multi_seg(const MultiArgs &ma, uint32_t slot)
{
    const uint32_t idx = reinterpret_cast<const_map_t *>(reinterpret_cast<uintptr_t>(ma.map))[__builtin_amdgcn_readfirstlane(slot)];
    return reinterpret_cast<const_seg_t *>(reinterpret_cast<uintptr_t>(ma.segs))[idx];
}


struct SrcRateUnmatch {
    static constexpr bool kIntegerValued = true;
    uint32_t e_cap;
    GroupDesc       g;
    const uint16_t *tabs;
    const uint32_t *nnn;
    const uint16_t *tab;
    const int8_t   *e;
    uint32_t        E, Nnn, K_;
    __device__ __forceinline__ void seg(const_seg_fwd_t &sg);
    __device__ __forceinline__ void init(uint32_t cb, uint32_t K)
    {
        const_u32x4_t *dp = reinterpret_cast<const_u32x4_t *>(reinterpret_cast<uintptr_t>(g.desc + cb));
        const u32x4_t  d0 = dp[0], d1 = dp[1];
        tab = tabs + (size_t)d0.w * 3 * K;
        Nnn = d1.x;
        K_  = K;
        e   = g.e_base + (size_t)d0.y * 64;
        E   = d0.z;
        hard = d1.y != 0;
    }
    bool hard;
    __device__ __forceinline__ bool hard_inputs() const { return hard; }
    __device__ __forceinline__ bool stage_e(int8_t *lds)
    {
        if (E + 16 > e_cap || E >= 0xFFFFu) return false;
        const uint32_t nq = E >> 4, tail = E & 15u;
        const uint4   *gp = reinterpret_cast<const uint4 *>(e);
        uint4         *l  = reinterpret_cast<uint4 *>(lds);
#pragma unroll 4
        for (uint32_t w = threadIdx.x; w < nq; w += blockDim.x) l[w] = gp[w];
        if (threadIdx.x == (nq & 63u)) {
            uint4 t = make_uint4(0, 0, 0, 0);
            if (tail) {
                t = gp[nq];
                uint32_t c[4] = {t.x, t.y, t.z, t.w};
#pragma unroll
                for (uint32_t k = 0; k < 4; k++) {
                    const int keep = (int)tail - 4 * (int)k;
                    c[k] = keep >= 4 ? c[k] : keep <= 0 ? 0u : (c[k] & ((1u << (8 * keep)) - 1u));
                }
                t = make_uint4(c[0], c[1], c[2], c[3]);
            }
            l[nq] = t;
        }
        __syncthreads();
        return true;
    }
    struct RankWords { uint4 raw[3][2]; };
    __device__ __forceinline__ void load_ranks(uint32_t u, int nvalid, RankWords &rw) const
    {
#pragma unroll
        for (int x = 0; x < 3; x++) {
            rw.raw[x][0] = rw.raw[x][1] = make_uint4(~0u, ~0u, ~0u, ~0u);
            if (nvalid > 0) {
                const uint4 *p = reinterpret_cast<const uint4 *>(tab + (size_t)x * K_ + 16 * (size_t)u);
                rw.raw[x][0] = p[0];
                if (nvalid > 8) rw.raw[x][1] = p[1];
            }
        }
    }
    template <typename Emit> __device__ __forceinline__ void gather16_staged(uint32_t el , uint32_t u, int nvalid, Emit emit) const
    {
        RankWords rw;
        load_ranks(u, nvalid, rw);
        gather16_staged(el, rw, emit);
    }
    template <typename Emit> __device__ __forceinline__ void gather16_staged(uint32_t el, const RankWords &rw, Emit emit) const
    {
        const uint4 (&raw)[3][2] = rw.raw;
#pragma unroll
        for (int x = 0; x < 3; x++) {
            const uint32_t w[8] = {raw[x][0].x, raw[x][0].y, raw[x][0].z, raw[x][0].w, raw[x][1].x, raw[x][1].y, raw[x][1].z, raw[x][1].w};
            uint32_t       r[16];
            int            acc[16];
#pragma unroll
            for (int k = 0; k < 16; k++) {
                r[k]   = (k & 1) ? (w[k >> 1] >> 16) : (w[k >> 1] & 0xFFFFu);
                acc[k] = lds_i8(el + min(r[k], E));
            }
            if (Nnn < E) {
                uint32_t rmin = r[0];
#pragma unroll
                for (int k = 1; k < 16; k++) rmin = min(rmin, r[k]);
                for (uint32_t base = Nnn; base < E; base += Nnn) {
                    if (!__any(rmin + base < E)) break;
#pragma unroll
                    for (int k = 0; k < 16; k++) acc[k] += lds_i8(el + min(r[k] + base, E));
                }
            }
            emit(x, acc);
        }
    }
    template <typename P, typename Emit> __device__ __forceinline__ void gather16(P ep, uint32_t u, int nvalid, Emit emit) const
    {
        RankWords rw;
        load_ranks(u, nvalid, rw);
        const uint4 (&raw)[3][2] = rw.raw;
#pragma unroll
        for (int x = 0; x < 3; x++) {
            uint32_t r[16];
            int      acc[16];
            {
                const uint32_t w[8] = {raw[x][0].x, raw[x][0].y, raw[x][0].z, raw[x][0].w, raw[x][1].x, raw[x][1].y, raw[x][1].z, raw[x][1].w};
#pragma unroll
                for (int k = 0; k < 16; k++) r[k] = (w[k >> 1] >> (16 * (k & 1))) & 0xFFFFu;
            }
#pragma unroll
            for (int k = 0; k < 16; k++) {
                const bool ok = k < nvalid && r[k] != 0xFFFFu && r[k] < E;
                const int  t  = (int)ep[ok ? r[k] : 0u];
                acc[k]        = ok ? t : 0;
                if (!ok) r[k] = 0xFFFFFFFFu - 65536u * 4u;
            }
            for (uint32_t base = Nnn; base < E; base += Nnn) {
#pragma unroll
                for (int k = 0; k < 16; k++) {
                    const uint32_t q = r[k] + base;
                    const int      t = (int)ep[q < E ? q : 0u];
                    acc[k] += (q < E) ? t : 0;
                }
            }
            emit(x, acc);
        }
    }
    static constexpr bool kPacked = false;
    static constexpr bool kIntPath = true;
    __device__ __forceinline__ void load16(uint32_t u, int nvalid, int (&v)[3][16], uint32_t e_lds, bool in_lds) const
    {
        auto emit = [&](int x, const int (&acc)[16]) {
#pragma unroll
            for (int k = 0; k < 16; k++) v[x][k] = acc[k];
        };
        if (in_lds) gather16_staged(e_lds, u, nvalid, emit);
        else        gather16(e, u, nvalid, emit);
    }
    __device__ __forceinline__ void load16_pk(uint32_t u, int nvalid, uint32_t (&vp)[3][8], uint32_t e_lds, bool in_lds) const
    {
        auto emit = [&](int x, const int (&acc)[16]) {
#pragma unroll
            for (int j = 0; j < 8; j++) vp[x][j] = __builtin_amdgcn_perm((uint32_t)acc[2 * j + 1], (uint32_t)acc[2 * j], 0x05040100u);
        };
        if (in_lds) gather16_staged(e_lds, u, nvalid, emit);
        else        gather16(e, u, nvalid, emit);
    }
    __device__ __forceinline__ bool window_ok() const { return Nnn + 48 <= e_cap; }
    __device__ __forceinline__ void gather_windowed_pk(uint32_t u, int nvalid, uint32_t (&vp)[3][8], int8_t *lds, uint32_t el) const
    {
        uint4 *l = reinterpret_cast<uint4 *>(lds);
        for (uint32_t base = 0; base < E; base += Nnn) {
            const uint32_t len = min(Nnn, E - base), shift = base & 15u, end = shift + len, nq = end >> 4, tail = end & 15u;
            const uint4   *gp = reinterpret_cast<const uint4 *>(e + (base - shift));
            RankWords rw;
            load_ranks(u, nvalid, rw);
            if (base) __syncthreads();
#pragma unroll 4
            for (uint32_t w = threadIdx.x; w < nq; w += blockDim.x) l[w] = gp[w];
            if (threadIdx.x == (nq & 63u)) {
                uint4 t = make_uint4(0, 0, 0, 0);
                if (tail) {
                    t = gp[nq];
                    uint32_t c[4] = {t.x, t.y, t.z, t.w};
#pragma unroll
                    for (uint32_t k = 0; k < 4; k++) {
                        const int keep = (int)tail - 4 * (int)k;
                        c[k] = keep >= 4 ? c[k] : keep <= 0 ? 0u : (c[k] & ((1u << (8 * keep)) - 1u));
                    }
                    t = make_uint4(c[0], c[1], c[2], c[3]);
                }
                l[nq] = t;
            }
            __syncthreads();
            if (nvalid > 0) {
#pragma unroll
                for (int x = 0; x < 3; x++) {
                    const uint32_t w[8] = {rw.raw[x][0].x, rw.raw[x][0].y, rw.raw[x][0].z, rw.raw[x][0].w, rw.raw[x][1].x, rw.raw[x][1].y, rw.raw[x][1].z, rw.raw[x][1].w};
                    int acc[16];
#pragma unroll
                    for (int k = 0; k < 16; k++) {
                        const uint32_t r = (k & 1) ? (w[k >> 1] >> 16) : (w[k >> 1] & 0xFFFFu);
                        acc[k] = lds_i8(el + shift + min(r, len));
                    }
#pragma unroll
                    for (int j = 0; j < 8; j++)
                        vp[x][j] = as_u32(as_v2s(vp[x][j]) + as_v2s(__builtin_amdgcn_perm((uint32_t)acc[2 * j + 1], (uint32_t)acc[2 * j], 0x05040100u)));
                }
            }
        }
    }
};
__device__ __forceinline__ void SrcRateUnmatch::seg(const_seg_fwd_t &sg)
{
    tabs = (const uint16_t *)sg.tabs; nnn = (const uint32_t *)sg.nnn; g.desc += sg.cb_base;
}
struct SrcRateUnmatchPk : SrcRateUnmatch { static constexpr bool kPacked = true; };

__device__ __forceinline__ uint32_t pack4u(uint32_t b0, uint32_t b1, uint32_t b2, uint32_t b3) { return b0 | (b1 << 8) | (b2 << 16) | (b3 << 24); }
__device__ __forceinline__ uint32_t bias4(uint32_t w) { return w ^ 0x80808080u; }
template <int K4> __device__ __forceinline__ uint32_t abs_sum2(uint32_t wa_biased, uint32_t wb_biased)
{
    return __builtin_amdgcn_msad_u8(wb_biased, 0x80u << (8 * K4), __builtin_amdgcn_msad_u8(wa_biased, 0x80u << (8 * K4), 0u));
}
__device__ __forceinline__ void abs_sum16(const uint4 &A, const uint4 &B, uint32_t (&w)[16], uint32_t &wmax)
{
    const uint32_t a[4] = {bias4(A.x), bias4(A.y), bias4(A.z), bias4(A.w)}, b[4] = {bias4(B.x), bias4(B.y), bias4(B.z), bias4(B.w)};
#pragma unroll
    for (int j = 0; j < 4; j++) {
        w[4 * j]     = abs_sum2<0>(a[j], b[j]);
        w[4 * j + 1] = abs_sum2<1>(a[j], b[j]);
        w[4 * j + 2] = abs_sum2<2>(a[j], b[j]);
        w[4 * j + 3] = abs_sum2<3>(a[j], b[j]);
        wmax = max(max(wmax, w[4 * j]), max(w[4 * j + 1], max(w[4 * j + 2], w[4 * j + 3])));
    }
}
__device__ __forceinline__ uint4 lookup16(uint32_t base, const uint32_t (&w)[16])
{
    uint32_t o[4];
#pragma unroll
    for (int j = 0; j < 4; j++) o[j] = pack4u(lds_u8(base + w[4 * j]), lds_u8(base + w[4 * j + 1]), lds_u8(base + w[4 * j + 2]), lds_u8(base + w[4 * j + 3]));
    return make_uint4(o[0], o[1], o[2], o[3]);
}
__device__ __forceinline__ uint4 gather16_bytes(uint32_t base, const uint32_t (&idx)[16]) { return lookup16(base, idx); }

template <typename Src, int NSLOT, bool MULTI = false>
#ifndef PREP_WPE
#define PREP_WPE 6
#endif
#ifndef PREP_WPE_PK
#define PREP_WPE_PK 6
#endif
__global__ __launch_bounds__(384) __attribute__((amdgpu_waves_per_eu(Src::kPacked ? PREP_WPE_PK : PREP_WPE, 8))) void k_turbo_prep(Src src, uint32_t K_arg, uint32_t n_cb_arg,
                                                    const uint16_t *__restrict__ pi_arg, PrepOut out, MultiArgs ma)
{
    static_assert(NSLOT == 1, "one unit per thread (K <= 6144 -> at most 384 units)");
    uint32_t K = K_arg, n_cb = n_cb_arg, bidx = blockIdx.x;
    size_t   seg_off = 0;
    const uint16_t *__restrict__ pi = pi_arg;
    if constexpr (MULTI) {
        const_seg_t &sg = multi_seg(ma, blockIdx.x >> 9);
        K = sg.K; n_cb = sg.n_cb; pi = (const uint16_t *)sg.pi; bidx = blockIdx.x - sg.wg_cb; seg_off = sg.arr_off;
        src.e_cap = sg.e_cap;
        src.seg(sg);
    }
    extern __shared__ __attribute__((aligned(16))) int8_t sm[];
    const uint32_t cb = xcd_cb(bidx, n_cb), tile = cb >> 6, lane = cb & 63, Kp = kpad64(K), n_units = Kp >> 4;
    const size_t   tile_off = seg_off + (size_t)tile * Kp * 64;
    if (cb >= n_cb) {
        if (MULTI && cb < ((n_cb + 63u) & ~63u) && threadIdx.x < n_units)
#pragma unroll
            for (int a = 0; a < 6; a++) *reinterpret_cast<uint4 *>(out.arr[a] + unit_off(tile_off, lane, threadIdx.x)) = make_uint4(0, 0, 0, 0);
        return;
    }
    int8_t        *qtab = sm + PREP_QTAB_AT, *qc = qtab + QTAB_HALF, *mtab1 = sm, *mtab2 = mtab1 + MTAB_N, *e_lds = sm + PREP_E_AT;
// ... 747 lines not shown
    if (nv > 0) {
        const uint32_t  iw[8] = {vraw.lo.x, vraw.lo.y, vraw.lo.z, vraw.lo.w, vraw.hi.x, vraw.hi.y, vraw.hi.z, vraw.hi.w};
        uint32_t        me[4], mo[4], bw[4];
#pragma unroll
        for (int j = 0; j < 4; j++) {
            const uint32_t i0 = iw[2 * j] & 0xFFFFu, i1 = iw[2 * j] >> 16, i2 = iw[2 * j + 1] & 0xFFFFu, i3 = iw[2 * j + 1] >> 16;
            const uint32_t ge = lds_u16(i0) | lds_u16(i2) << 16, go = lds_u16(i1) | lds_u16(i3) << 16;
            me[j] = as_u32((s0e[j] + as_v2s(ge)) >> 15);
            mo[j] = as_u32((s0o[j] + as_v2s(go)) >> 15);
            bw[j] = (me[j] & 0x00010001u) | (mo[j] & 0x00010001u) << 8;
        }
        if (GROUP) {
            if (!(nv == 16 && 16 * u >= F)) {
#pragma unroll
                for (int j = 0; j < 4; j++) {
                    auto ok = [&](int k) { return (k < nv && 16 * u + k >= F) ? 0xFFFFu : 0u; };
                    me[j] &= ok(4 * j) | ok(4 * j + 2) << 16;
                    mo[j] &= ok(4 * j + 1) | ok(4 * j + 3) << 16;
                }
            }
            const uint32_t GS = 0x864CFBu << 8;
            uint32_t       w = crc_w0;
#pragma unroll
            for (int k = 15; k >= 0; k--) {
                const int      j = k >> 2;
                const uint32_t m = (k & 3) == 0 ? (uint32_t)__builtin_amdgcn_sbfe(me[j], 0, 1) : (k & 3) == 1 ? (uint32_t)__builtin_amdgcn_sbfe(mo[j], 0, 1)
                                 : (k & 3) == 2 ? (uint32_t)((int)me[j] >> 31) : (uint32_t)((int)mo[j] >> 31);
                crc ^= w & m;
                if (k > 0) w = (w << 1) ^ ((uint32_t)((int)w >> 31) & GS);
            }
        }
        const uint4 pk = make_uint4(bw[0], bw[1], bw[2], bw[3]);
        if (GROUP) *reinterpret_cast<uint4 *>(bits + 16 * u) = pk;
        else {
            uint2 *o = reinterpret_cast<uint2 *>(c_bits + (size_t)cb * K + 16 * u);
            o[0] = make_uint2(pk.x, pk.y);
            if (nv > 8) o[1] = make_uint2(pk.z, pk.w);
        }
    }
    if (GROUP) {
        crc = wave_xor_u(crc);
        __syncthreads();
        if ((threadIdx.x & 63) == 0) red_u[threadIdx.x >> 6] = crc;
        __syncthreads();
        crc = 0;
        for (uint32_t w = 0; w < (blockDim.x >> 6); w++) crc ^= red_u[w];
        if (threadIdx.x == 0) g.status[alloc] = (crc == 0) ? 0  : 2 ;
        uint8_t *o = g.out_bits + (size_t)alloc * g.out_stride;
        if (g.packed && ((F | tbs) & 7u) == 0) {
            const uint32_t nby = tbs >> 3, nw = nby >> 2;
            auto byte_at = [&](uint32_t m) -> uint32_t {
                const uint2 w = *reinterpret_cast<const uint2 *>(bits + F + 8 * m);
                return (((w.x * 0x08040201u) >> 24) & 0xFu) << 4 | (((w.y * 0x08040201u) >> 24) & 0xFu);
            };
            for (uint32_t m = threadIdx.x; m < nw; m += blockDim.x)
                reinterpret_cast<uint32_t *>(o)[m] = byte_at(4 * m) | byte_at(4 * m + 1) << 8 | byte_at(4 * m + 2) << 16 | byte_at(4 * m + 3) << 24;
            for (uint32_t m = 4 * nw + threadIdx.x; m < nby; m += blockDim.x) o[m] = (uint8_t)byte_at(m);
        } else if (g.packed) {
            for (uint32_t m = threadIdx.x; m < (tbs + 7) >> 3; m += blockDim.x) {
                uint32_t v = 0;
                for (uint32_t b = 0; b < 8; b++) v = v << 1 | ((8 * m + b < tbs) ? ((uint32_t)bits[F + 8 * m + b] & 1u) : 0u);
                o[m] = (uint8_t)v;
            }
        } else if ((F & 3u) == 0) {
            const uint32_t nq = tbs >> 2;
            const uint32_t *bw = reinterpret_cast<const uint32_t *>(bits + F);
            for (uint32_t m = threadIdx.x; m < nq; m += blockDim.x) reinterpret_cast<uint32_t *>(o)[m] = bw[m];
            for (uint32_t m = 4 * nq + threadIdx.x; m < tbs; m += blockDim.x) o[m] = (uint8_t)bits[m + F];
        } else
            for (uint32_t m = threadIdx.x; m < tbs; m += blockDim.x) o[m] = (uint8_t)bits[m + F];
    }
}

__global__ __launch_bounds__(256) void k_cb_desc(GroupDesc g, uint32_t n_cb, const uint32_t *__restrict__ nnn, CbDesc *__restrict__ out)
{
    const uint32_t cb = blockIdx.x * blockDim.x + threadIdx.x;
    if (cb >= n_cb) return;
    const uint32_t a = g.cb_alloc[cb], txm = g.allocs[a].tx_mode;
    const uint32_t combo = g.ul ? 8u + (g.allocs[a].rv_idx & 3u)
                                : ((g.allocs[a].rv_idx & 3u) << 1) | ((txm == 3 || txm == 4 || txm == 8 || txm == 9) ? 1u : 0u);
    CbDesc d;
    d.alloc = a; d.e_off = g.e_off[a]; d.E = g.e_len[a]; d.combo = combo; d.Nnn = nnn[combo];
    d.hard  = (g.allocs[a].mod_type >= 2 && d.E <= d.Nnn) ? 1u : 0u;
    d.tbs   = g.allocs[a].tbs; d.pad = 0;
    out[cb] = d;
}

__global__ __launch_bounds__(256) void k_cb_desc_multi(GroupDesc g, uint32_t n_cb, const KSeg *__restrict__ segs, uint32_t n_seg, CbDesc *__restrict__ out)
{
    const uint32_t cb = blockIdx.x * blockDim.x + threadIdx.x;
    if (cb >= n_cb) return;
    uint32_t lo = 0, hi = n_seg;
    while (hi - lo > 1) {
        const uint32_t mid = (lo + hi) >> 1;
        if (segs[mid].cb_base <= cb) lo = mid; else hi = mid;
    }
    const uint32_t a = g.cb_alloc[cb], txm = g.allocs[a].tx_mode;
    const uint32_t combo = g.ul ? 8u + (g.allocs[a].rv_idx & 3u)
                                : ((g.allocs[a].rv_idx & 3u) << 1) | ((txm == 3 || txm == 4 || txm == 8 || txm == 9) ? 1u : 0u);
    CbDesc d;
    d.alloc = a; d.e_off = g.e_off[a]; d.E = g.e_len[a]; d.combo = combo; d.Nnn = segs[lo].nnn[combo];
    d.hard  = (g.allocs[a].mod_type >= 2 && d.E <= d.Nnn) ? 1u : 0u;
    d.tbs   = g.allocs[a].tbs; d.pad = 0;
    out[cb] = d;
}

__global__ __launch_bounds__(256) void k_rm_rank_table(uint32_t K, uint16_t *__restrict__ tabs, uint32_t *__restrict__ nnn)
{
    const uint32_t combo = blockIdx.y, t = blockIdx.x * blockDim.x + threadIdx.x;
    RmGeom rm;
    if (combo < 8) rm.init(K + 4, (combo & 1) ? 3 : 1, combo >> 1);
    else           rm.init(K + 4, 1, combo - 8, 1, 1, 1, false);
    if (t == 0) nnn[combo] = rm.Nnn;
    if (t >= 3 * K) return;
    const uint32_t x = t / K, i = t - x * K;
    uint32_t p, c;
    rm.pos_cnt(i, (int)x, p, c);
    uint32_t k = 0xFFFFu;
    if (p < rm.N_cb) k = (p >= rm.k0m) ? c - rm.cnt_k0 : rm.Nnn - rm.cnt_k0 + c;
    tabs[(size_t)combo * 3 * K + t] = (uint16_t)k;
}

struct RmParams { uint32_t D, E, C, tx_mode, N_soft, M_dl_harq, limited, rv; };

__global__ __launch_bounds__(256) void k_rate_unmatch_f32(const float *__restrict__ e, RmParams pr, uint32_t n_cb,
                                                          float *__restrict__ d)
{
    RmGeom rm;
    rm.init(pr.D, pr.tx_mode, pr.rv, pr.N_soft, pr.M_dl_harq, pr.C, pr.limited != 0);
    const uint32_t cb = blockIdx.y;
    const float   *eb = e + (size_t)cb * pr.E;
    float         *db = d + (size_t)cb * 3 * pr.D;
    for (uint32_t t = blockIdx.x * blockDim.x + threadIdx.x; t < 3 * pr.D; t += gridDim.x * blockDim.x) {
        const uint32_t i = t / 3;
        const int      x = (int)(t - 3 * i);
        const uint32_t p = rm.pos(i, x);
        float          v = (float)RX_NULL_AS_INT;
        if (p < rm.N_cb) {
            const uint32_t c = rm.cnt(p);
            uint32_t       k = (p >= rm.k0m) ? c - rm.cnt_k0 : rm.Nnn - rm.cnt_k0 + c;
            if (k < pr.E) {
                v = eb[k];
                for (k += rm.Nnn; k < pr.E; k += rm.Nnn)
                    if (eb[k] != (float)RX_NULL_AS_INT) v += eb[k];
            }
        }
        db[t] = v;
    }
}

__global__ __launch_bounds__(256) void k_rm_to_i8(GroupDesc g, uint32_t K, uint32_t n_cb, const uint16_t *__restrict__ tabs, const uint32_t *__restrict__ nnn,
                                                  int8_t *__restrict__ d_soft, uint32_t e_cap)
{
    extern __shared__ __attribute__((aligned(16))) int8_t e_lds[];
    __shared__ RmGeom rm_s;
    const uint32_t cb = blockIdx.x, D = K + 4, a = g.cb_alloc[cb], txm = g.allocs[a].tx_mode, rv = g.allocs[a].rv_idx & 3u;
    if (threadIdx.x == 0) {
        if (g.ul) rm_s.init(D, 1, rv, 1, 1, 1, false);
        else      rm_s.init(D, txm, rv);
    }
    const uint32_t combo = g.ul ? 8u + rv : (rv << 1) | ((txm == 3 || txm == 4 || txm == 8 || txm == 9) ? 1u : 0u);
    const uint16_t *tab = tabs + (size_t)combo * 3 * K;
    const uint32_t Nnn = nnn[combo], E = g.e_len[a];
    const int8_t  *e = g.e_base + (size_t)g.e_off[a] * 64;
    int8_t        *db = d_soft + (size_t)cb * 3 * D;
    const bool     staged = E + 16 <= e_cap && E < 0xFFFFu;
    if (staged) {
        const uint32_t nq = (E + 15) >> 4;
        for (uint32_t w = threadIdx.x; w < nq; w += blockDim.x) reinterpret_cast<uint4 *>(e_lds)[w] = reinterpret_cast<const uint4 *>(e)[w];
        __syncthreads();
        for (uint32_t k = E + threadIdx.x; k < ((E + 16) & ~15u); k += blockDim.x) e_lds[k] = 0;
    }
    __syncthreads();
    auto sum_at = [&](uint32_t k) -> int {
        int v = 0;
        if (staged) {
            v = e_lds[min(k, E)];
            for (uint32_t q = k + Nnn; q < E; q += Nnn) v += e_lds[q];
        } else if (k != 0xFFFFu) {
            for (; k < E; k += Nnn) v += e[k];
        }
        return max(-127, min(127, v));
    };
    for (uint32_t i0 = 4 * threadIdx.x; i0 < K; i0 += 4 * blockDim.x) {
        uint32_t r[3][4];
#pragma unroll
// ... 170 lines not shown
        d_desc = (CbDesc *)(base + N_BYTE_ARRAYS * arr_bytes + 3 * (arr_bytes / 2) + 3 * (arr_bytes / 8));
        po.arr[0] = arr[AX0]; po.arr[1] = arr[AX1]; po.arr[2] = arr[AX2];
        po.arr[3] = arr[AI0]; po.arr[4] = arr[AM1]; po.arr[5] = arr[AM2];
        s1.p[0] = {arr[AX1], arr[AX0], sgn[0], dec[0]};
        s1.p[1] = s1.p[0];
        pa.M1 = arr[AM1]; pa.S1 = sgn[0]; pa.X2 = arr[AX2]; pa.out[0] = arr[AI1]; pa.out[1] = arr[AM3];
        s23.p[0] = {arr[AX2], arr[AI0], sgn[1], dec[1]};
        s23.p[1] = {arr[AX2], arr[AI1], sgn[2], dec[2]};
        va = {arr[AX0], arr[AM1], arr[AM2], arr[AM3], sgn[0], sgn[1], sgn[2]};
    }
};

template <typename Src, bool GROUP>
static int turbo_ref_run(mi_lte_ctx *ctx, Src src, uint32_t K, uint32_t n_cb, uint8_t *d_c_bits, GroupDesc gd, uint32_t e_cap = 0)
{
    TurboTables tb;
    int         rc = mi_ctx_turbo_tables(ctx, K, 0, &tb);
    if (rc != MI_LTE_OK) return rc;
    static const bool lds_ok = no_static_lds({(const void *)k_turbo_prep<Src, 1>, (const void *)k_turbo_perm<1>, (const void *)k_turbo_vote<GROUP, 1>});
    if (!lds_ok) { ctx->err = "turbo kernels were built with static LDS: absolute LDS addressing is invalid"; return MI_LTE_ERR_HIP; }
    const size_t n_tiles = (n_cb + 63) / 64, Kp = kpad64(K), arr_bytes = n_tiles * Kp * 64;
    rc = mi_ctx_reserve_scratch(ctx, ref_scratch_bytes(arr_bytes, n_tiles * 64));
    if (rc != MI_LTE_OK) return rc;
    const RefScratch sc(ctx->scratch, arr_bytes);
    const bool small = n_cb <= ctx->siso_small_max;
    if (n_cb % 64 && !small)
        MI_HIP_CHECK(ctx, hipMemsetAsync(sc.base, 0, N_BYTE_ARRAYS * arr_bytes, ctx->stream));

    if constexpr (GROUP) {
        gd.desc = src.g.desc = sc.d_desc;
        MI_LAUNCH(ctx, "k_cb_desc", k_cb_desc, dim3((n_cb + 255) / 256), dim3(256), 0, gd, n_cb, (const uint32_t *)src.nnn, sc.d_desc);
    }
    const uint32_t cb_threads = cb_width(K);
    MI_LAUNCH(ctx, "k_turbo_prep", (k_turbo_prep<Src, 1>), dim3(cb_grid(n_cb)), dim3(cb_threads), prep_lds_bytes(Kp, e_cap), src, K, n_cb, tb.d_pi, sc.po, MultiArgs{});

    auto lds_of = [&](uint32_t gpw) { return siso_small_lds_bytes(gpw, Kp); };
    if (small)
        MI_LAUNCH(ctx, "k_turbo_siso_small", k_turbo_siso_small<false>, dim3((n_cb + gpw_of(n_cb) - 1) / gpw_of(n_cb)), dim3(64), lds_of(gpw_of(n_cb)), sc.s1, K, n_cb, 0u,
                  gpw_of(n_cb), MultiArgs{});
    else
        MI_LAUNCH(ctx, "k_turbo_siso", (k_turbo_siso<false, 0>), dim3(((n_tiles + 1) / 2 + 3) / 4), dim3(256), 0, sc.s1, K, (uint32_t)n_tiles, MultiArgs{}, (const uint32_t *)nullptr);

    MI_LAUNCH(ctx, "k_turbo_perm", k_turbo_perm<1>, dim3(perm_grid_of(n_cb)), dim3(cb_threads), MTAB_N + Kp + 32, sc.pa, K, n_cb, tb.d_pi, MultiArgs{});

    if (small)
        MI_LAUNCH(ctx, "k_turbo_siso_small", k_turbo_siso_small<false>, dim3((2 * n_cb + gpw_of(2 * n_cb) - 1) / gpw_of(2 * n_cb)), dim3(64), lds_of(gpw_of(2 * n_cb)), sc.s23, K,
                  n_cb, 1u, gpw_of(2 * n_cb), MultiArgs{});
    else
        MI_LAUNCH(ctx, "k_turbo_siso", (k_turbo_siso<false, 1>), dim3((n_tiles + 3) / 4), dim3(256), 0, sc.s23, K, (uint32_t)n_tiles, MultiArgs{}, (const uint32_t *)nullptr);

    MI_LAUNCH(ctx, "k_turbo_vote", (k_turbo_vote<GROUP, 1>), dim3(cb_grid(n_cb)), dim3(cb_threads), 3 * Kp + 64, sc.va, K, n_cb, tb.d_inv2, d_c_bits, gd, MultiArgs{});
    MI_HIP_CHECK(ctx, hipGetLastError());
    ctx->last_kernels = "k_turbo_prep:1,k_turbo_siso:2,k_turbo_perm:1,k_turbo_vote:1";
    return MI_LTE_OK;
}

template <typename T>
static int turbo_ref_batch(mi_lte_ctx *ctx, const T *d_soft, uint32_t K, uint32_t n_cb, uint8_t *d_c_bits)
{
    SrcDirect<T> src{0, d_soft, nullptr};
    GroupDesc    none{};
    return turbo_ref_run<SrcDirect<T>, false>(ctx, src, K, n_cb, d_c_bits, none);
}

static int rm_rank_tables(mi_lte_ctx *ctx, uint32_t K, RmTables *out)
{
    auto it = ctx->rm_tables.find(K);
    if (it == ctx->rm_tables.end()) {
        RmTables t;
        MI_HIP_CHECK(ctx, hipMalloc((void **)&t.d_tabs, sizeof(uint16_t) * 12 * 3 * K));
        MI_HIP_CHECK(ctx, hipMalloc((void **)&t.d_nnn, sizeof(uint32_t) * 12));
        ctx->owned.push_back(t.d_tabs);
        ctx->owned.push_back(t.d_nnn);
        MI_LAUNCH(ctx, "k_rm_rank_table", k_rm_rank_table, dim3((3 * K + 255) / 256, 12), dim3(256), 0, K, t.d_tabs, t.d_nnn);
        MI_HIP_CHECK(ctx, hipGetLastError());
        it = ctx->rm_tables.emplace(K, t).first;
    }
    *out = it->second;
    return MI_LTE_OK;
}

static GroupDesc group_desc(const mi_lte_ctx *ctx, const MiDecodeIO &io, uint32_t cb_base = 0)
{
    return {io.d_allocs, io.d_cb_alloc + cb_base, io.d_e, io.d_e_off, io.d_e_len, io.d_out_bits, io.out_stride, io.d_status, ctx->d_crc_tab, io.ul ? 1u : 0u, io.packed ? 1u : 0u};
}

static int mi_turbo_ref_group(mi_lte_ctx *ctx, const MiKGroup &gr, const MiDecodeIO &io)
{
    int rc = mi_ctx_crc_table(ctx);
    if (rc != MI_LTE_OK) return rc;
    const GroupDesc gd = group_desc(ctx, io, gr.cb_base);
    RmTables rt;
    rc = rm_rank_tables(ctx, gr.K, &rt);
    if (rc != MI_LTE_OK) return rc;
    SrcRateUnmatch src;
    src.g    = gd;
    src.tabs = rt.d_tabs;
    src.nnn  = rt.d_nnn;
    const uint32_t cap = stage_cap(gr.e_max);
    src.e_cap          = prep_stages(gr.K, cap) ? cap : 0;
    if (mi_turbo_ref_multi_takes(gr.K, gr.e_max)) {
        SrcRateUnmatchPk pk;
        static_cast<SrcRateUnmatch &>(pk) = src;
        return turbo_ref_run<SrcRateUnmatchPk, true>(ctx, pk, gr.K, gr.n_cb, nullptr, gd, src.e_cap);
    }
    return turbo_ref_run<SrcRateUnmatch, true>(ctx, src, gr.K, gr.n_cb, nullptr, gd, src.e_cap);
}

static int mi_turbo_ref_multi(mi_lte_ctx *ctx, const MiKGroup *groups, uint32_t n_groups, const MiDecodeIO &io, MiMultiCache *cache)
{
    if (!groups || n_groups == 0 || n_groups > 0xFFFF || !cache) return MI_LTE_ERR_INVALID_ARG;
    int rc = mi_ctx_crc_table(ctx);
    if (rc != MI_LTE_OK) return rc;
    static const bool lds_ok = no_static_lds({(const void *)k_turbo_prep<SrcRateUnmatchPk, 1, true>, (const void *)k_turbo_perm<1, true>, (const void *)k_turbo_vote<true, 1, true>});
    if (!lds_ok) { ctx->err = "turbo kernels were built with static LDS: absolute LDS addressing is invalid"; return MI_LTE_ERR_HIP; }
    const bool same = cache->built_for.size() == n_groups && memcmp(cache->built_for.data(), groups, sizeof(MiKGroup) * n_groups) == 0;
    if (!same) {
        cache->built_for.clear();
        cache->geom = MiMultiGeom{};
        std::vector<std::pair<TurboTables, RmTables>> tabs(n_groups);
        for (uint32_t i = 0; i < n_groups; i++)
            if ((rc = mi_ctx_turbo_tables(ctx, groups[i].K, 0, &tabs[i].first)) != MI_LTE_OK || (rc = rm_rank_tables(ctx, groups[i].K, &tabs[i].second)) != MI_LTE_OK) return rc;
        MiMultiPlan plan;
        const char *why = nullptr;
        if ((rc = mi_turbo_multi_plan(groups, n_groups, &plan, &why)) != MI_LTE_OK) {
            if (why) ctx->err = why;
            return rc;
        }
        for (uint32_t i = 0; i < n_groups; i++) {
            KSeg &sg = plan.segs[i];
            sg.pi = (decltype(sg.pi))tabs[i].first.d_pi; sg.inv2 = (decltype(sg.inv2))tabs[i].first.d_inv2;
            sg.tabs = (decltype(sg.tabs))tabs[i].second.d_tabs; sg.nnn = (decltype(sg.nnn))tabs[i].second.d_nnn;
        }
        const size_t seg_bytes = plan.geom.map_off, map_bytes = (sizeof(uint32_t) * plan.map.size() + 15) & ~(size_t)15, need = seg_bytes + map_bytes;
        if (need > cache->cap) {
            MI_HIP_CHECK(ctx, hipStreamSynchronize(ctx->stream));
            if (cache->d_tab) (void)hipFree(cache->d_tab);
            cache->d_tab = nullptr; cache->cap = 0;
            MI_HIP_CHECK(ctx, hipMalloc(&cache->d_tab, need + need / 4));
            cache->cap = need + need / 4;
        }
        std::vector<uint8_t> blob(need, 0);
        memcpy(blob.data(), plan.segs.data(), seg_bytes);
        memcpy(blob.data() + seg_bytes, plan.map.data(), sizeof(uint32_t) * plan.map.size());
        MI_H2D(ctx, cache->d_tab, blob.data(), need);
        cache->geom = plan.geom;
        cache->built_for.assign(groups, groups + n_groups);
    }
    const MiMultiGeom &G = cache->geom;
    const size_t A = G.arr_bytes;
    rc = mi_ctx_reserve_scratch(ctx, ref_scratch_bytes(A, G.n_slots));
    if (rc != MI_LTE_OK) return rc;
    const RefScratch sc(ctx->scratch, A);
    const KSeg     *d_segs = (const KSeg *)cache->d_tab;
    const uint32_t *d_map  = (const uint32_t *)((const uint8_t *)cache->d_tab + G.map_off);

    GroupDesc gd = group_desc(ctx, io);
    gd.desc = sc.d_desc;
    MI_LAUNCH(ctx, "k_cb_desc", k_cb_desc_multi, dim3((G.n_slots + 255) / 256), dim3(256), 0, gd, G.n_slots, d_segs, n_groups, sc.d_desc);
    SrcRateUnmatchPk src;
    src.g = gd; src.tabs = nullptr; src.nnn = nullptr; src.e_cap = 0;
    for (int c = 0; c < NCLS; c++)
        if (G.grid_cb[c]) {
            if (G.one_size[c] >= 0) {
                const MiKGroup &gr = groups[G.one_size[c]];
                TurboTables tb;
                RmTables    rt;
                if ((rc = mi_ctx_turbo_tables(ctx, gr.K, 0, &tb)) != MI_LTE_OK || (rc = rm_rank_tables(ctx, gr.K, &rt)) != MI_LTE_OK) return rc;
                SrcRateUnmatchPk s1 = src;
                s1.tabs = rt.d_tabs; s1.nnn = rt.d_nnn; s1.g.desc = sc.d_desc + gr.cb_base; s1.e_cap = G.e_cap_one[c];
                PrepOut p1 = sc.po;
                for (int a = 0; a < 6; a++) p1.arr[a] += G.off_one[c];
                MI_LAUNCH(ctx, "k_turbo_prep", (k_turbo_prep<SrcRateUnmatchPk, 1, false>), dim3(G.grid_cb[c]), dim3(64 * (c + 1)), G.lds_prep[c], s1, gr.K, gr.n_cb, (const uint16_t *)tb.d_pi,
                          p1, MultiArgs{});
                continue;
            }
            MI_LAUNCH(ctx, "k_turbo_prep", (k_turbo_prep<SrcRateUnmatchPk, 1, true>), dim3(G.grid_cb[c]), dim3(64 * (c + 1)), G.lds_prep[c], src, 0u, 0u, (const uint16_t *)nullptr, sc.po,
                      (MultiArgs{d_segs, d_map + G.map_cb[c]}));
        }
    const bool small = G.n_slots <= ctx->siso_small_max;
    auto lds_small = [&](uint32_t gpw) { return siso_small_lds_bytes(gpw, G.kp_all); };
    if (small)
        MI_LAUNCH(ctx, "k_turbo_siso_small", k_turbo_siso_small<true>, dim3(G.n_ws1), dim3(64), lds_small(G.gpw1), sc.s1, 0u, 0u, 0u, G.gpw1, (MultiArgs{d_segs, d_map + G.map_ws1}));
    else
// ... 124 lines not shown
```

### openlte_amd/csrc/turbo_plan.hpp

```cpp
#pragma once

#include <cstddef>
#include <cstdint>
#include <vector>

#ifdef __HIPCC__
#define MI_HD __host__ __device__
#else
#define MI_HD
#endif
#ifdef __clang__
#define MI_GLOBAL_AS __attribute__((address_space(1)))
#else
#define MI_GLOBAL_AS
#endif

namespace turbo_geom {

MI_HD inline uint32_t kpad64(uint32_t K) { return (K + 63u) & ~63u; }

MI_HD inline uint32_t xcd_chunk(uint32_t n_cb) { return ((((n_cb + 63u) >> 6) + 7u) >> 3) << 6; }
MI_HD inline uint32_t xcd_cb(uint32_t b, uint32_t n_cb) { return (b & 7u) * xcd_chunk(n_cb) + (b >> 3); }
inline uint32_t cb_grid(uint32_t n_cb) { return 8 * xcd_chunk(n_cb); }

constexpr int NCLS = 6;
inline uint32_t cb_width(uint32_t K) { return ((kpad64(K) >> 4) + 63u) & ~63u; }
inline int      cb_class(uint32_t K) { return (int)(cb_width(K) >> 6) - 1; }

constexpr uint32_t PERM_BLOCKS = 4;
inline uint32_t perm_grid_of(uint32_t n_cb) { return ((cb_grid(n_cb) + PERM_BLOCKS - 1) / PERM_BLOCKS + 7u) & ~7u; }

constexpr uint32_t SMALL_G = 8;
inline uint32_t gpw_of(uint32_t n_tr) { return n_tr <= 2048 ? 1u : n_tr <= 4096 ? 2u : n_tr <= 8192 ? 4u : SMALL_G; }
inline size_t   siso_small_lds_bytes(uint32_t gpw, size_t Kp) { return sizeof(uint32_t) * gpw * (64 * 4 * 2 + (Kp >> 5) * 4); }

constexpr uint32_t QTAB_N = 4096;
constexpr uint32_t QTAB_HALF = 2048;
constexpr uint32_t MTAB_N = 256;
constexpr uint32_t PREP_RED_AT = 2 * MTAB_N, PREP_E_AT = PREP_RED_AT + 64, PREP_QTAB_AT = PREP_E_AT, PREP_Q0_AT = PREP_QTAB_AT + QTAB_N;
MI_HD constexpr uint32_t prep_lds_bytes(uint32_t Kp, uint32_t e_cap) { return PREP_E_AT + (e_cap > QTAB_N + Kp ? e_cap : QTAB_N + Kp); }
inline uint32_t stage_cap(uint32_t e_max_bytes) { return (e_max_bytes + 16u + 63u) & ~63u; }
inline bool prep_stages(uint32_t K, uint32_t cap) { return prep_lds_bytes(kpad64(K), cap) <= 48 * 1024; }
inline uint32_t merged_e_cap(uint32_t K, uint32_t e_max_bytes)
{
    const uint32_t cap = stage_cap(e_max_bytes), cap_w = (uint32_t)((15 * (size_t)(K + 4) / 4 + 64 + 63) & ~(size_t)63);
    return prep_stages(K, cap) ? (kpad64(K) <= 1024 ? (cap < cap_w ? cap : cap_w) : cap) : cap_w;
}

inline bool mi_turbo_ref_multi_takes(uint32_t K, uint32_t e_max_bytes) { return (e_max_bytes + (3 * K - 81) - 1) / (3 * K - 81) <= 258; }

constexpr int    N_BYTE_ARRAYS = 8;
constexpr size_t CB_DESC_BYTES = 32;
inline size_t ref_scratch_bytes(size_t arr_bytes, size_t n_slots) { return N_BYTE_ARRAYS * arr_bytes + 3 * (arr_bytes / 2) + 3 * (arr_bytes / 8) + ((n_slots + 63) & ~(size_t)63) * CB_DESC_BYTES; }

}

struct MiKGroup { uint32_t K, n_cb, cb_base, e_max; };

struct KSeg {
    uint32_t        K, n_cb, cb_base, n_tiles;
    uint32_t        wg_cb;
    uint32_t        wg_perm, perm_grid;
    uint32_t        e_cap;
    uint32_t        wv1, wv23;
    uint64_t        arr_off;
    MI_GLOBAL_AS const uint16_t *pi, *inv2, *tabs;
    MI_GLOBAL_AS const uint32_t *nnn;
    uint32_t        ws1, ws23;
    uint64_t        pad;
};
static_assert(sizeof(KSeg) == 96, "KSeg is read with scalar loads: keep it a multiple of 16 bytes");
struct MultiArgs { const KSeg *segs; const uint32_t *map; };

struct MiMultiGeom {
    uint64_t arr_bytes = 0;
    uint32_t n_slots = 0, n_wv1 = 0, n_wv23 = 0;
    uint32_t grid_cb[6] = {0}, grid_perm[6] = {0}, lds_prep[6] = {0}, kp_max[6] = {0};
    uint32_t map_cb[6] = {0}, map_perm[6] = {0}, map_wv1 = 0, map_wv23 = 0;
    uint32_t ord_wv1 = 0, ord_wv23 = 0, n_ord1 = 0, n_ord23 = 0;
    uint32_t siso_pad1 = 0, siso_pad23 = 0;
    int      one_size[6] = {-1, -1, -1, -1, -1, -1};
    uint64_t off_one[6] = {0}; uint32_t e_cap_one[6] = {0};
    uint32_t map_ws1 = 0, map_ws23 = 0, n_ws1 = 0, n_ws23 = 0, gpw1 = 1, gpw23 = 1, kp_all = 0;
    size_t   map_off = 0;
};

struct MiMultiPlan { std::vector<KSeg> segs; std::vector<uint32_t> map; MiMultiGeom geom; };
int mi_turbo_multi_plan(const MiKGroup *groups, uint32_t n_groups, MiMultiPlan *out, const char **err);
```

### openlte_amd/lib.py

```python
import ctypes as C
import os
import subprocess

import numpy as np

_HERE = os.path.dirname(os.path.abspath(__file__))
_LIB = None

SOFT_F32, SOFT_I8, SOFT_I16 = 0, 1, 2
TURBO_REF, TURBO_BCJR, TURBO_BCJR_BLOCK, TURBO_BCJR_EARLY = 0, 1, 2, 3
_SOFT_OF_DTYPE = {np.dtype(np.float32): SOFT_F32, np.dtype(np.int8): SOFT_I8, np.dtype(np.int16): SOFT_I16}


IQ_I8, IQ_F32_PLANAR = 0, 1
IQ_ALL_ROWS = 0x100
CE_COMPACT = 0x200


class DlCfg(C.Structure):
    _fields_ = [("fft_size", C.c_uint32), ("N_rb_dl", C.c_uint32), ("N_ant", C.c_uint32), ("sample_format", C.c_uint32)]


class UlCfg(C.Structure):
    _fields_ = [(n, C.c_uint32) for n in ("group_assignment_pusch", "group_hopping_enabled", "sequence_hopping_enabled",
# ... 1261 lines not shown
        return PdcchSearchPlan(self, cfg, cells, sizes, rntis, phich_res, any_cce)

    def pusch_plan(self, cfg, ulcfg, unit_subfr_num, unit_n_id_cell, allocs, uci=None):
        return PuschPlan(self, cfg, ulcfg, unit_subfr_num, unit_n_id_cell, allocs, uci=uci)

    def pusch_plan_3gpp(self, cfg, ulcfg, unit_subfr_num, unit_n_id_cell, allocs, uci=None):
        return PuschPlan(self, cfg, ulcfg, unit_subfr_num, unit_n_id_cell, allocs, spec=True, uci=uci)

    def cqi_decode_batch(self, soft, descs):
        soft = np.ascontiguousarray(soft, np.int8)
        arr = (CqiDesc * len(descs))(*[CqiDesc(off, q, o, 0) for off, q, o in descs])
        for d in arr:
            if 1 <= d.O <= CQI_MAX_BITS and 1 <= d.Q_cqi <= CQI_MAX_Q and d.off % 2 == 0 and d.off + d.Q_cqi > len(soft):
                raise ValueError("cqi_decode_batch: run at %d + %d past the %d soft bits" % (d.off, d.Q_cqi, len(soft)))
        d_soft, d_desc, d_out = self.alloc(max(soft.nbytes, 2)), self.alloc(C.sizeof(arr)), self.alloc(C.sizeof(CqiResult) * len(descs))
        try:
            if soft.nbytes:
                d_soft.upload(soft)
            self._check(self.L.mi_lte_memcpy_h2d(self.h, d_desc.ptr, C.addressof(arr), C.sizeof(arr)))
            self._check(self.L.mi_lte_cqi_decode_batch(self.h, d_soft.ptr, d_desc.ptr, len(descs), d_out.ptr))
            rec = (CqiResult * len(descs))()
            self._check(self.L.mi_lte_memcpy_d2h(self.h, C.addressof(rec), d_out.ptr, C.sizeof(rec)))
            return [r.as_dict() for r in rec]
        finally:
            d_soft.free()
            d_desc.free()
            d_out.free()

    def pdsch_plan(self, cfg, n_pdcch_symbs, allocs):
        return PdschPlan(self, cfg, n_pdcch_symbs, allocs)

    def pdsch_plan_3gpp(self, cfg, n_pdcch_symbs, allocs, n_soft, m_dl_harq=8):
        return PdschPlan(self, cfg, n_pdcch_symbs, allocs, dlsch=DlschCfg(n_soft, m_dl_harq))

    def harq_pool(self, n_buf, max_tbs=75376):
        return HarqPool(self, n_buf, max_tbs)

    def pdsch_plan_dynamic(self, cfg, max_alloc, max_soft_bytes):
        return PdschPlan(self, cfg, 0, None, max_alloc, max_soft_bytes)

    def iq_to_planar(self, d_iq, n_samples, d_i, d_q):
        self._check(self.L.mi_lte_iq_i8_to_planar(self.h, d_iq.ptr, n_samples, d_i.ptr, d_q.ptr))

    def freq_shift(self, d_i, d_q, first_index, n_samples, freq_offset, fs):
        self._check(self.L.mi_lte_freq_shift_run(self.h, d_i.ptr, d_q.ptr, first_index, n_samples, float(freq_offset), int(fs)))

    def turbo_decode_dev(self, d_soft, soft_type, K, n_cb, d_out, mode=TURBO_REF, n_iter=8, qpp_spec=False):
        self._check(self.L.mi_lte_turbo_decode_batch(self.h, d_soft.ptr, soft_type, K, n_cb, mode, n_iter,
                                                     1 if qpp_spec else 0, d_out.ptr))

    def turbo_decode(self, soft, K, mode=TURBO_REF, n_iter=8, qpp_spec=False):
        soft = np.ascontiguousarray(soft)
        assert soft.ndim == 2 and soft.shape[1] == 3 * (K + 4), soft.shape
        n_cb = soft.shape[0]
        d_in = self.to_device(soft)
        d_out = self.alloc(n_cb * K)
        try:
            self.turbo_decode_dev(d_in, _SOFT_OF_DTYPE[soft.dtype], K, n_cb, d_out, mode, n_iter, qpp_spec)
            return d_out.download(np.uint8).reshape(n_cb, K)
        finally:
            d_in.free()
            d_out.free()

    def device_copy_rate(self, nbytes=1 << 30, reps=10):
        out = C.c_double()
        self._check(self.L.mi_lte_device_copy_rate(self.h, C.c_size_t(nbytes), reps, C.byref(out)))
        return out.value

    def device_copy_rates(self):
        out = (C.c_double * 3)()
        self._check(self.L.mi_lte_device_copy_rates(self.h, out))
        return tuple(round(v, 1) for v in out)

    def turbo_early_exit_iterations(self):
        n, ni = C.c_uint32(), C.c_uint32()
        out = np.zeros(1 << 16, np.uint32)
        self._check(self.L.mi_lte_turbo_early_exit_iterations(self.h, out.ctypes.data, len(out), C.byref(n), C.byref(ni)))
        return out[:n.value].copy()

    def set_turbo_merged(self, on=True):
        self.L.mi_lte_set_turbo_merged.argtypes = [C.c_void_p, C.c_uint32]
        self._check(self.L.mi_lte_set_turbo_merged(self.h, 1 if on else 0))

    def set_turbo_small_batch(self, n_cb_max):
        self._check(self.L.mi_lte_set_turbo_small_batch(self.h, int(n_cb_max)))

    def close(self):
        if getattr(self, "h", None):
            self.L.mi_lte_ctx_destroy(self.h)
            self.h = None

    def __del__(self):
        try:
            self.close()
        except Exception:
            pass
```

Baseline: 2.928 million subframes/s.

## Pack hard-decision QAM soft bits to one bit per LLR between demod and turbo

For 16/64QAM allocations on the REF demap and REF turbo path, the demodulator now stores only sign bits, one bit per soft bit instead of one int8, after scrambling in LDS. The turbo rate-unmatch staging expands them back to +/-127 bytes on the fly. A debug tap kernel expands the buffer in place when soft bits are requested. The aim is to cut HBM write and read traffic for the soft-bit buffer by about 8x. The cost is extra pack and unpack ALU work, larger demod LDS use, and more code-path complexity.

```diff
diff --git a/include/mi_lte.h b/include/mi_lte.h
--- a/include/mi_lte.h
+++ b/include/mi_lte.h
@@ -159,6 +159,7 @@
 
 int mi_lte_set_turbo_small_batch(mi_lte_ctx *ctx, uint32_t n_cb_max);
 int mi_lte_set_turbo_merged(mi_lte_ctx *ctx, uint32_t on);
+int mi_lte_set_soft_packed(mi_lte_ctx *ctx, uint32_t on);
 
 int mi_lte_rate_unmatch_turbo_batch(mi_lte_ctx *ctx, const float *d_e_bits, uint32_t N_e_bits, uint32_t D,
                                     uint32_t N_codeblocks, uint32_t tx_mode, uint32_t N_soft, uint32_t M_dl_harq,
diff --git a/openlte_amd/csrc/chain.hip b/openlte_amd/csrc/chain.hip
--- a/openlte_amd/csrc/chain.hip
+++ b/openlte_amd/csrc/chain.hip
@@ -5,6 +5,7 @@
 #include "plan_core.hpp"
 #include "phy_dev.hpp"
 #include "demap_llr.h"
+#include "soft_pack.h"
 
 namespace {
 
@@ -79,7 +80,7 @@
                                                      const uint32_t *__restrict__ subfr_num, const uint32_t *__restrict__ n_id_cell,
                                                      GoldTables gt, int8_t *__restrict__ e_base, const uint32_t *__restrict__ e_off,
                                                      uint32_t *__restrict__ e_len, uint32_t max_pairs, uint32_t max_words,
-                                                     uint32_t e_lds_cap)
+                                                     uint32_t e_lds_cap, uint32_t pack)
 {
     extern __shared__ __attribute__((aligned(16))) uint32_t smu[];
     __shared__ uint2 qam_lut[64];
@@ -123,9 +124,16 @@
     };
     int8_t    *e_lds  = reinterpret_cast<int8_t *>(cw + max_words);
     const bool via_lds = N_bits <= e_lds_cap;
-    auto run = [&](auto modc) {
+    const bool pk = pack && al.mod_type >= 2;
+    auto run = [&](auto modc, auto pkc) {
     constexpr uint32_t MOD = decltype(modc)::value, QM = MOD == 3 ? 6 : MOD == 2 ? 4 : MOD == 1 ? 2 : 1;
-    constexpr bool     QAM = MOD >= 2;
+    constexpr bool     QAM = MOD >= 2, PK = decltype(pkc)::value;
+    static_assert(QAM || !PK, "only hard-decision modulations are packed");
+    auto each_dst = [&](auto f) {
+        if constexpr (PK) f(e_lds);
+        else if (via_lds) f(e_lds);
+        else f(e);
+    };
     auto put_bits = [&](auto *dst, uint32_t idx, const int8_t (&b)[6]) {
         const uint32_t n0 = idx * QM, w = n0 >> 5, sh = n0 & 31;
         const uint32_t c = __builtin_amdgcn_alignbit(cw[w + 1], cw[w], sh);
@@ -150,8 +158,14 @@
             *reinterpret_cast<uint16_t *>(dst + n0 + 4) = (uint16_t)v.y;
         }
     };
+    auto put_mask = [&](auto *dst, uint32_t idx, uint32_t neg) {
+        const uint32_t n0 = QM == 4 ? idx << 2 : __umul24(idx, 6u), w = n0 >> 5, sh = n0 & 31;
+        const uint32_t c  = __builtin_amdgcn_alignbit(cw[w + 1], cw[w], sh);
+        reinterpret_cast<uint8_t *>(dst)[idx] = (uint8_t)((neg ^ c) & (QM == 4 ? 15u : 63u));
+    };
     auto put_symbol = [&](auto *dst, uint32_t idx, float nr, float ni, float den) {
-        if constexpr (QAM) put_qam(dst, idx, qam_neg_bits_nodiv<MOD>(nr, ni, den));
+        if constexpr (PK) put_mask(dst, idx, qam_neg_bits_nodiv<MOD>(nr, ni, den));
+        else if constexpr (QAM) put_qam(dst, idx, qam_neg_bits_nodiv<MOD>(nr, ni, den));
         else {
             int8_t b[6] = {0, 0, 0, 0, 0, 0};
             demap_symbol<true>(nr / den, ni / den, MOD, b);
@@ -206,7 +220,7 @@
                 }
             }
         };
-        if (via_lds) body(e_lds); else body(e);
+        each_dst(body);
     } else if (ONE_PORT) {
         constexpr int UNR = 4;
         const uint32_t q_thr = threadIdx.x / 12, j = threadIdx.x - 12 * q_thr, below = (1u << j) - 1u;
@@ -237,7 +251,7 @@
                 }
             }
         };
-        if (via_lds) body(e_lds); else body(e);
+        each_dst(body);
     } else
     for (uint32_t i = threadIdx.x; i < n_grp; i += blockDim.x) {
         float n_re[4], n_im[4], den[4];
@@ -271,19 +285,45 @@
             n_re[3] = -h3r * y2r - h3i * y2i + h1r * y3r + h1i * y3i;
             n_im[3] = -(-h3r * y2i + h3i * y2r - h1r * y3i + h1i * y3r);
         }
-        for (uint32_t p = 0; p < N_ant; p++) {
-            if (via_lds) put_symbol(e_lds, i * N_ant + p, n_re[p], n_im[p], den[p]);
-            else         put_symbol(e, i * N_ant + p, n_re[p], n_im[p], den[p]);
+#pragma unroll
+        for (uint32_t p = 0; p < 4; p++) {
+            if (p >= N_ant) break;
+            if (PK || via_lds) put_symbol(e_lds, i * N_ant + p, n_re[p], n_im[p], den[p]);
+            else               put_symbol(e, i * N_ant + p, n_re[p], n_im[p], den[p]);
         }
     }
     };
     switch (al.mod_type) {
-    case 0:  run(std::integral_constant<uint32_t, 0>{}); break;
-    case 1:  run(std::integral_constant<uint32_t, 1>{}); break;
-    case 2:  run(std::integral_constant<uint32_t, 2>{}); break;
-    default: run(std::integral_constant<uint32_t, 3>{}); break;
-    }
-    if (via_lds) {
+    case 0:  run(std::integral_constant<uint32_t, 0>{}, std::false_type{}); break;
+    case 1:  run(std::integral_constant<uint32_t, 1>{}, std::false_type{}); break;
+    case 2:  if (pk) run(std::integral_constant<uint32_t, 2>{}, std::true_type{}); else run(std::integral_constant<uint32_t, 2>{}, std::false_type{}); break;
+    default: if (pk) run(std::integral_constant<uint32_t, 3>{}, std::true_type{}); else run(std::integral_constant<uint32_t, 3>{}, std::false_type{}); break;
+    }
+    if (pk) {
+        __syncthreads();
+        const uint32_t nd = (N_bits + 31) >> 5, ng = (M_symb + 15) >> 4;
+        uint32_t      *eo = reinterpret_cast<uint32_t *>(e);
+        for (uint32_t gi = threadIdx.x; gi < ng; gi += blockDim.x) {
+            const uint4    m4 = reinterpret_cast<const uint4 *>(e_lds)[gi];
+            const uint32_t m[4] = {m4.x, m4.y, m4.z, m4.w}, nv = min(16u, M_symb - 16 * gi);
+            if (Qm == 4) {
+                uint32_t o[2];
+                soft_pack16<4>(m, nv, o);
+                const uint32_t d0 = 2 * gi;
+                if (d0 + 2 <= nd) *reinterpret_cast<uint2 *>(eo + d0) = make_uint2(o[0], o[1]);
+                else eo[d0] = o[0];
+            } else {
+                uint32_t o[3];
+                soft_pack16<6>(m, nv, o);
+                const uint32_t d0 = 3 * gi;
+                if (d0 + 3 <= nd) { eo[d0] = o[0]; eo[d0 + 1] = o[1]; eo[d0 + 2] = o[2]; }
+                else {
+                    eo[d0] = o[0];
+                    if (d0 + 1 < nd) eo[d0 + 1] = o[1];
+                }
+            }
+        }
+    } else if (via_lds) {
         __syncthreads();
         const uint32_t nq = (N_bits + 15) >> 4;
         for (uint32_t w = threadIdx.x; w < nq; w += blockDim.x) reinterpret_cast<uint4 *>(e)[w] = reinterpret_cast<const uint4 *>(e_lds)[w];
@@ -410,6 +450,23 @@
         for (uint32_t w = threadIdx.x; w < nq; w += blockDim.x) reinterpret_cast<uint4 *>(e)[w] = reinterpret_cast<const uint4 *>(e_lds)[w];
     } else
         per_mod(e);
+}
+
+__global__ __launch_bounds__(256) void k_soft_expand(const mi_lte_pdsch_alloc *__restrict__ allocs, int8_t *__restrict__ e_base, const uint32_t *__restrict__ e_off,
+                                                     const uint32_t *__restrict__ e_len, uint32_t max_words)
+{
+    extern __shared__ __attribute__((aligned(16))) uint32_t smu[];
+    const uint32_t a_idx = blockIdx.x;
+    if (allocs[a_idx].mod_type < 2) return;
+    const uint32_t E = e_len[a_idx], nd = min((E + 31) >> 5, max_words), nq = min((E + 15) >> 4, 2 * max_words);
+    int8_t *e = e_base + (size_t)e_off[a_idx] * 64;
+    for (uint32_t w = threadIdx.x; w < nd; w += blockDim.x) smu[w] = reinterpret_cast<const uint32_t *>(e)[w];
+    __syncthreads();
+    for (uint32_t q = threadIdx.x; q < nq; q += blockDim.x) {
+        uint32_t w[4];
+        soft_stage_quad(smu, q, min(16u, E - 16 * q), w);
+        reinterpret_cast<uint4 *>(e)[q] = make_uint4(w[0], w[1], w[2], w[3]);
+    }
 }
 
 }
@@ -433,6 +490,9 @@
     MiDlsch3   *g3 = nullptr;
     uint32_t    demap = MI_LTE_DEMAP_REF;
     float       demap_gain = 0.0f, *d_llr_gain = nullptr;
+    uint32_t            max_words_lo = 0, max_symb_hi = 0;
+    mutable mi_lte_ctx *tap_ctx = nullptr;
+    mutable bool        tap_packed = false;
 };
 
 static void plan_set_stride(mi_lte_pdsch_plan *pl)
@@ -450,7 +510,8 @@
     const mi_lte_dl_cfg *cfg = &pl->cfg;
     pl->cfi          = N_pdcch_symbs;
     pl->core.n_alloc = n_alloc;
-    pl->max_pairs = pl->max_words = pl->max_tbs = 0;
+    pl->max_pairs = pl->max_words = pl->max_tbs = pl->max_words_lo = pl->max_symb_hi = 0;
+    pl->tap_packed = false;
     pl->core.groups.clear();
     for (uint32_t a = 0; a < n_alloc; a++) {
         const mi_lte_pdsch_alloc &al = h_allocs[a];
@@ -472,6 +533,8 @@
         const uint32_t pairs = (14 - cfi) * al.N_prb, e_max = pairs * 12 * Qm;
         pl->max_pairs = std::max(pl->max_pairs, 14 * al.N_prb);
         pl->max_words = std::max(pl->max_words, (e_max + 31) / 32);
+        if (al.mod_type >= 2) pl->max_symb_hi = std::max(pl->max_symb_hi, pairs * 12);
+        else pl->max_words_lo = std::max(pl->max_words_lo, (e_max + 31) / 32);
         e_bits[a]     = e_max;
     }
     if (pl->max_words > 4095) {
@@ -714,6 +777,14 @@
 int mi_lte_pdsch_plan_soft_bits(const mi_lte_pdsch_plan *pl, uint32_t alloc, const int8_t **d_e, const uint32_t **d_len)
 {
     if (!pl || alloc >= pl->core.n_alloc || !d_e || !d_len) return MI_LTE_ERR_INVALID_ARG;
+    if (pl->tap_packed) {
+        mi_lte_ctx *ctx = pl->tap_ctx;
+        MI_HIP_CHECK(ctx, hipSetDevice(ctx->device));
+        hipLaunchKernelGGL(k_soft_expand, dim3(pl->core.n_alloc), dim3(256), sizeof(uint32_t) * (pl->max_words + 4u), ctx->stream, pl->core.d_allocs, pl->core.d_e,
+                           pl->core.d_e_off, pl->core.d_e_len, pl->max_words);
+        MI_HIP_CHECK(ctx, hipGetLastError());
+        pl->tap_packed = false;
+    }
     *d_e   = pl->core.d_e + (size_t)pl->core.h_e_off[alloc] * 64;
     *d_len = pl->core.d_e_len + alloc;
     return MI_LTE_OK;
@@ -756,17 +827,17 @@
 
 }
 
-static int pdsch_demod(mi_lte_ctx *ctx, mi_lte_pdsch_plan *pl, const float *d_subframes, const uint32_t *d_subfr_num, const uint32_t *d_n_id_cell)
+static int pdsch_demod(mi_lte_ctx *ctx, mi_lte_pdsch_plan *pl, const float *d_subframes, const uint32_t *d_subfr_num, const uint32_t *d_n_id_cell, bool pack)
 {
     MI_HIP_CHECK(ctx, hipSetDevice(ctx->device));
     int rc = mi_ctx_gold_tables(ctx);
     if (rc != MI_LTE_OK) return rc;
     DemodGeom  g{pl->cfg.N_rb_dl, pl->cfg.N_ant, pl->cfi, (uint32_t)mi_lte_subframe_floats(pl->cfg.N_ant)};
     GoldTables gt{ctx->d_gold_x1, ctx->d_gold_x2b, ctx->gold_words};
-    const uint32_t words_al = (pl->max_words + 1u + 3u) & ~3u, e_bytes = (pl->max_words * 32 + 63u) & ~63u;
+    const uint32_t words_al = (pl->max_words + 1u + 3u) & ~3u, e_bytes = ((pack ? pl->max_words_lo : pl->max_words) * 32 + 63u) & ~63u;
     const uint32_t e_cap = (e_bytes <= 32 * 1024) ? e_bytes : 0;
     const uint32_t pairs_al = ((2 * (pl->max_pairs + 1) + 3u) & ~3u);
-    const size_t lds = sizeof(uint32_t) * ((size_t)pairs_al + words_al) + e_cap;
+    const size_t lds = sizeof(uint32_t) * ((size_t)pairs_al + words_al) + std::max(e_cap, pack ? (pl->max_symb_hi + 15u) & ~15u : 0u);
     uint32_t threads = 256;
     if (const char *ev = getenv("MI_LTE_PDSCH_THREADS")) {
         const int t = atoi(ev);
@@ -774,7 +845,7 @@
     }
     auto launch = [&](auto kernel) {
         MI_LAUNCH(ctx, "k_pdsch_demod", kernel, dim3(pl->core.n_alloc), dim3(threads), lds, d_subframes, g, pl->core.d_allocs, d_subfr_num, d_n_id_cell, gt,
-                  pl->core.d_e, pl->core.d_e_off, pl->core.d_e_len, pl->max_pairs, words_al, e_cap);
+                  pl->core.d_e, pl->core.d_e_off, pl->core.d_e_len, pl->max_pairs, words_al, e_cap, pack ? 1u : 0u);
     };
     if (pl->demap == MI_LTE_DEMAP_MAXLOG) {
         float auto_t = (float)MI_LTE_DEMAP_AUTO_T;
@@ -801,8 +872,11 @@
         if ((rc = mi_dlsch3_harq_check(ctx, pl->g3, pool, h_bind)) != MI_LTE_OK) return rc;
     }
     if (pl->core.n_alloc == 0) { ctx->err = "the dynamic plan holds no allocations (mi_lte_pdsch_plan_assign)"; return MI_LTE_ERR_INVALID_ARG; }
-    if ((rc = pdsch_demod(ctx, pl, d_subframes, d_subfr_num, d_n_id_cell)) != MI_LTE_OK) return rc;
-    const MiDecodeIO io = pl->core.io(d_out_bits, d_status, false);
+    bool pack = ctx->soft_packed && !pl->g3 && !mi_is_bcjr(pl->decoder) && pl->demap == MI_LTE_DEMAP_REF;
+    for (const MiKGroup &gr : pl->core.groups) pack = pack && turbo_geom::mi_turbo_ref_reads_packed(gr.K, gr.e_max);
+    if ((rc = pdsch_demod(ctx, pl, d_subframes, d_subfr_num, d_n_id_cell, pack)) != MI_LTE_OK) return rc;
+    pl->tap_ctx = ctx; pl->tap_packed = pack;
+    const MiDecodeIO io = pl->core.io(d_out_bits, d_status, false, pack);
     if (pl->g3) {
         rc = mi_dlsch3_run(ctx, pl->g3, pool, h_bind, io, pl->decoder, pl->n_iter);
         if (rc == MI_LTE_OK && pl->demap == MI_LTE_DEMAP_MAXLOG) ctx->last_kernels.replace(0, strlen("k_pdsch_demod"), "k_pdsch_demod_llr");
diff --git a/openlte_amd/csrc/ctx.cc b/openlte_amd/csrc/ctx.cc
--- a/openlte_amd/csrc/ctx.cc
+++ b/openlte_amd/csrc/ctx.cc
@@ -36,6 +36,7 @@
     mi_lte_ctx *ctx = new mi_lte_ctx();
     ctx->device     = device;
     if (const char *e = getenv("MI_LTE_NO_MERGED_DECODE")) ctx->merged_decode = atoi(e) == 0;
+    if (const char *e = getenv("MI_LTE_NO_SOFT_PACK")) ctx->soft_packed = atoi(e) == 0;
     hipDeviceProp_t prop;
     if (hipSetDevice(device) != hipSuccess || hipGetDeviceProperties(&prop, device) != hipSuccess) {
         delete ctx;
@@ -87,6 +88,13 @@
 {
     if (!ctx) return MI_LTE_ERR_INVALID_ARG;
     ctx->merged_decode = on != 0;
+    return MI_LTE_OK;
+}
+
+int mi_lte_set_soft_packed(mi_lte_ctx *ctx, uint32_t on)
+{
+    if (!ctx) return MI_LTE_ERR_INVALID_ARG;
+    ctx->soft_packed = on != 0;
     return MI_LTE_OK;
 }
 
diff --git a/openlte_amd/csrc/ctx.hpp b/openlte_amd/csrc/ctx.hpp
--- a/openlte_amd/csrc/ctx.hpp
+++ b/openlte_amd/csrc/ctx.hpp
@@ -46,6 +46,7 @@
     bool               bcjr_block_lds_set = false;
     uint32_t           siso_small_max = 4096;
     bool               merged_decode = true;
+    bool               soft_packed = true;
     void              *h_small = nullptr, *d_small = nullptr;
     void              *h_bounce = nullptr, *d_bounce = nullptr;
     hipEvent_t         ev_bounce[2] = {nullptr, nullptr};
diff --git a/openlte_amd/csrc/plan_core.hpp b/openlte_amd/csrc/plan_core.hpp
--- a/openlte_amd/csrc/plan_core.hpp
+++ b/openlte_amd/csrc/plan_core.hpp
@@ -19,6 +19,7 @@
     int32_t        *d_status;
     uint32_t        out_stride;
     bool            ul, packed;
+    bool            soft_packed;
 };
 
 struct MiPlanCore {
@@ -36,7 +37,7 @@
 
     hipError_t allocate(uint32_t n_alloc_max, size_t e_bytes_max, void *d_desc_block = nullptr);
     void       release();
-    MiDecodeIO io(uint8_t *d_out_bits, int32_t *d_status, bool ul) const { return {d_allocs, d_cb_alloc, d_e_off, d_e_len, d_e, d_out_bits, d_status, out_stride, ul, packed != 0}; }
+    MiDecodeIO io(uint8_t *d_out_bits, int32_t *d_status, bool ul, bool soft_packed = false) const { return {d_allocs, d_cb_alloc, d_e_off, d_e_len, d_e, d_out_bits, d_status, out_stride, ul, packed != 0, soft_packed}; }
 };
 
 int   mi_turbo_ref_dispatch(mi_lte_ctx *ctx, const MiKGroup *groups, uint32_t n_groups, const MiDecodeIO &io, MiMultiCache *cache);
diff --git a/openlte_amd/csrc/soft_pack.h b/openlte_amd/csrc/soft_pack.h
--- /dev/null
+++ b/openlte_amd/csrc/soft_pack.h
@@ -0,0 +1,50 @@
+#pragma once
+#include <stdint.h>
+
+#if defined(__HIPCC__)
+#define SOFT_PACK_FN __host__ __device__ __forceinline__
+#define SOFT_PACK_UNROLL _Pragma("unroll")
+#else
+#define SOFT_PACK_FN inline
+#define SOFT_PACK_UNROLL
+#endif
+
+SOFT_PACK_FN uint32_t soft_expand4(uint32_t nib) { return (((nib & 15u) * 0x00204081u) & 0x01010101u) * 2u + 0x7F7F7F7Fu; }
+
+SOFT_PACK_FN void soft_expand16(uint32_t bits, uint32_t (&w)[4])
+{
+    SOFT_PACK_UNROLL
+    for (int k = 0; k < 4; k++) w[k] = soft_expand4(bits >> (4 * k));
+}
+
+SOFT_PACK_FN void soft_keep_bytes(uint32_t (&w)[4], uint32_t keep)
+{
+    SOFT_PACK_UNROLL
+    for (uint32_t k = 0; k < 4; k++) {
+        const int kp = (int)keep - 4 * (int)k;
+        w[k] = kp >= 4 ? w[k] : kp <= 0 ? 0u : (w[k] & ((1u << (8 * kp)) - 1u));
+    }
+}
+
+SOFT_PACK_FN void soft_stage_quad(const void *slot, uint32_t q, uint32_t keep, uint32_t (&w)[4])
+{
+    soft_expand16(((const uint16_t *)slot)[q], w);
+    if (keep < 16) soft_keep_bytes(w, keep);
+}
+
+template <uint32_t QM> SOFT_PACK_FN void soft_pack16(const uint32_t (&m)[4], uint32_t n_valid, uint32_t (&out)[QM / 2])
+{
+    static_assert(QM == 4 || QM == 6, "16QAM or 64QAM");
+    uint64_t lo = 0, hi = 0;
+    SOFT_PACK_UNROLL
+    for (uint32_t s = 0; s < 16; s++) {
+        const uint32_t p = s * QM;
+        const uint64_t v = s < n_valid ? (uint64_t)((m[s >> 2] >> (8 * (s & 3))) & ((1u << QM) - 1u)) : 0u;
+        if (p < 64) lo |= v << p;
+        if (p < 64 && p + QM > 64) hi |= v >> (64 - p);
+        if (p >= 64) hi |= v << (p - 64);
+    }
+    out[0] = (uint32_t)lo;
+    out[1] = (uint32_t)(lo >> 32);
+    if (QM == 6) out[QM / 2 - 1] = (uint32_t)hi;
+}
diff --git a/openlte_amd/csrc/turbo.hip b/openlte_amd/csrc/turbo.hip
--- a/openlte_amd/csrc/turbo.hip
+++ b/openlte_amd/csrc/turbo.hip
@@ -6,6 +6,7 @@
 
 #include "plan_core.hpp"
 #include "turbo_swar.h"
+#include "soft_pack.h"
 
 using namespace turbo_geom;
 
@@ -236,7 +237,7 @@
     }
 };
 
-struct CbDesc { uint32_t alloc, e_off, E, combo, Nnn, hard, tbs, pad; };
+struct CbDesc { uint32_t alloc, e_off, E, combo, Nnn, hard, tbs, pk; };
 
 struct GroupDesc {
     const mi_lte_pdsch_alloc *allocs;
@@ -250,6 +251,7 @@
     const uint32_t *crc_tab;
     uint32_t        ul;
     uint32_t        packed;
+    uint32_t        soft_pk;
     const CbDesc   *desc;
 };
 
@@ -282,15 +284,29 @@
         e   = g.e_base + (size_t)d0.y * 64;
         E   = d0.z;
         hard = d1.y != 0;
-    }
-    bool hard;
+        pk   = d1.w != 0;
+    }
+    bool hard, pk;
     __device__ __forceinline__ bool hard_inputs() const { return hard; }
+    __device__ __forceinline__ static uint4 packed_quad(const int8_t *slot, uint32_t q, uint32_t keep)
+    {
+        uint32_t w[4];
+        soft_stage_quad(slot, q, keep, w);
+        return make_uint4(w[0], w[1], w[2], w[3]);
+    }
     __device__ __forceinline__ bool stage_e(int8_t *lds)
     {
         if (E + 16 > e_cap || E >= 0xFFFFu) return false;
         const uint32_t nq = E >> 4, tail = E & 15u;
         const uint4   *gp = reinterpret_cast<const uint4 *>(e);
         uint4         *l  = reinterpret_cast<uint4 *>(lds);
+        if (pk) {
+#pragma unroll 4
+            for (uint32_t w = threadIdx.x; w < nq; w += blockDim.x) l[w] = packed_quad(e, w, 16u);
+            if (threadIdx.x == (nq & 63u)) l[nq] = tail ? packed_quad(e, nq, tail) : make_uint4(0, 0, 0, 0);
+            __syncthreads();
+            return true;
+        }
 #pragma unroll 4
         for (uint32_t w = threadIdx.x; w < nq; w += blockDim.x) l[w] = gp[w];
         if (threadIdx.x == (nq & 63u)) {
@@ -417,6 +433,14 @@
             RankWords rw;
             load_ranks(u, nvalid, rw);
             if (base) __syncthreads();
+            if (pk) {
+                const uint32_t q0 = (base - shift) >> 4;
+#pragma unroll 1
+                for (uint32_t w = threadIdx.x; w <= nq; w += blockDim.x) {
+                    const uint32_t keep = w < nq ? 16u : tail;
+                    l[w] = keep ? packed_quad(e, q0 + w, keep) : make_uint4(0, 0, 0, 0);
+                }
+            } else {
 #pragma unroll 4
             for (uint32_t w = threadIdx.x; w < nq; w += blockDim.x) l[w] = gp[w];
             if (threadIdx.x == (nq & 63u)) {
@@ -432,6 +456,7 @@
                     t = make_uint4(c[0], c[1], c[2], c[3]);
                 }
                 l[nq] = t;
+            }
             }
             __syncthreads();
             if (nvalid > 0) {
@@ -1345,7 +1370,7 @@
     CbDesc d;
     d.alloc = a; d.e_off = g.e_off[a]; d.E = g.e_len[a]; d.combo = combo; d.Nnn = nnn[combo];
     d.hard  = (g.allocs[a].mod_type >= 2 && d.E <= d.Nnn) ? 1u : 0u;
-    d.tbs   = g.allocs[a].tbs; d.pad = 0;
+    d.tbs   = g.allocs[a].tbs; d.pk = (g.soft_pk && g.allocs[a].mod_type >= 2) ? 1u : 0u;
     out[cb] = d;
 }
 
@@ -1364,7 +1389,7 @@
     CbDesc d;
     d.alloc = a; d.e_off = g.e_off[a]; d.E = g.e_len[a]; d.combo = combo; d.Nnn = segs[lo].nnn[combo];
     d.hard  = (g.allocs[a].mod_type >= 2 && d.E <= d.Nnn) ? 1u : 0u;
-    d.tbs   = g.allocs[a].tbs; d.pad = 0;
+    d.tbs   = g.allocs[a].tbs; d.pk = (g.soft_pk && g.allocs[a].mod_type >= 2) ? 1u : 0u;
     out[cb] = d;
 }
 
@@ -1701,7 +1726,7 @@
 
 static GroupDesc group_desc(const mi_lte_ctx *ctx, const MiDecodeIO &io, uint32_t cb_base = 0)
 {
-    return {io.d_allocs, io.d_cb_alloc + cb_base, io.d_e, io.d_e_off, io.d_e_len, io.d_out_bits, io.out_stride, io.d_status, ctx->d_crc_tab, io.ul ? 1u : 0u, io.packed ? 1u : 0u};
+    return {io.d_allocs, io.d_cb_alloc + cb_base, io.d_e, io.d_e_off, io.d_e_len, io.d_out_bits, io.out_stride, io.d_status, ctx->d_crc_tab, io.ul ? 1u : 0u, io.packed ? 1u : 0u, io.soft_packed ? 1u : 0u};
 }
 
 static int mi_turbo_ref_group(mi_lte_ctx *ctx, const MiKGroup &gr, const MiDecodeIO &io)
@@ -1719,6 +1744,7 @@
     const uint32_t cap = stage_cap(gr.e_max);
     src.e_cap          = prep_stages(gr.K, cap) ? cap : 0;
     if (mi_turbo_ref_multi_takes(gr.K, gr.e_max)) {
+        if (io.soft_packed && !src.e_cap) src.e_cap = merged_e_cap(gr.K, gr.e_max);
         SrcRateUnmatchPk pk;
         static_cast<SrcRateUnmatch &>(pk) = src;
         return turbo_ref_run<SrcRateUnmatchPk, true>(ctx, pk, gr.K, gr.n_cb, nullptr, gd, src.e_cap);
diff --git a/openlte_amd/csrc/turbo_plan.hpp b/openlte_amd/csrc/turbo_plan.hpp
--- a/openlte_amd/csrc/turbo_plan.hpp
+++ b/openlte_amd/csrc/turbo_plan.hpp
@@ -48,6 +48,7 @@
 }
 
 inline bool mi_turbo_ref_multi_takes(uint32_t K, uint32_t e_max_bytes) { return (e_max_bytes + (3 * K - 81) - 1) / (3 * K - 81) <= 258; }
+inline bool mi_turbo_ref_reads_packed(uint32_t K, uint32_t e_max_bytes) { return mi_turbo_ref_multi_takes(K, e_max_bytes) || prep_stages(K, stage_cap(e_max_bytes)); }
 
 constexpr int    N_BYTE_ARRAYS = 8;
 constexpr size_t CB_DESC_BYTES = 32;
diff --git a/openlte_amd/lib.py b/openlte_amd/lib.py
--- a/openlte_amd/lib.py
+++ b/openlte_amd/lib.py
@@ -1367,6 +1367,10 @@
         self.L.mi_lte_set_turbo_merged.argtypes = [C.c_void_p, C.c_uint32]
         self._check(self.L.mi_lte_set_turbo_merged(self.h, 1 if on else 0))
 
+    def set_soft_packed(self, on=True):
+        self.L.mi_lte_set_soft_packed.argtypes = [C.c_void_p, C.c_uint32]
+        self._check(self.L.mi_lte_set_soft_packed(self.h, 1 if on else 0))
+
     def set_turbo_small_batch(self, n_cb_max):
         self._check(self.L.mi_lte_set_turbo_small_batch(self.h, int(n_cb_max)))
 
```

After: 2.970 million subframes/s, median of 6. +1.4%, better.
